# newton-physics/newton

Hardware: NVIDIA H100
Metric: env_steps_per_sec (higher is better)
Workload: dtype f32

## Files before the change

newton_b200/build.py:

```python

from __future__ import annotations

import os
import subprocess
import sys

HERE = os.path.dirname(os.path.abspath(__file__))
CSRC = os.path.join(HERE, "csrc")
LIB = os.path.join(HERE, "libnewton_b200.so")
LIB_FAST = os.path.join(HERE, "libnewton_b200_fast.so")
STRICT_FLAGS = ["-fmad=false", "-DNB2_STRICT_FP=1"]
SOURCES = ["nb2_api.cu", "nb2_collide.cu", "nb2_xpbd.cu", "nb2_featherstone.cu", "nb2_selection.cu", "nb2_peer.cu", "nb2_match.cu"]
NVCC_FLAGS = [
    "-gencode", "arch=compute_90a,code=sm_90a", "-lineinfo", "-O3", "-std=c++17", "--expt-relaxed-constexpr",
    "-Xcompiler", "-fPIC", "-Xcompiler", "-O2",
]


def _nvcc() -> str:
    for c in (os.environ.get("NVCC"), "/usr/local/cuda/bin/nvcc", "nvcc"):
        if c and (os.path.isabs(c) and os.path.exists(c) or not os.path.isabs(c)):
            return c
    return "nvcc"


def needs_build() -> bool:
    if not os.path.exists(LIB):
        return True
    t = os.path.getmtime(LIB)
    deps = [os.path.join(CSRC, f) for f in os.listdir(CSRC)] + [os.path.join(HERE, "..", "include", "newton_b200.h")]
    return any(os.path.getmtime(p) > t for p in deps)


def build(force: bool = False, verbose: bool = False) -> str:
    if not force and not needs_build() and os.path.exists(LIB_FAST):
        return LIB
    procs = []
    variants = ((LIB, ".o", STRICT_FLAGS), (LIB_FAST, ".fast.o", []))
    for _lib_path, suffix, extra in variants:
        flags = NVCC_FLAGS + extra
        if verbose:
            flags = flags + ["-Xptxas", "-v"]
        for src in SOURCES:
            obj = os.path.join(CSRC, src.replace(".cu", suffix))
            cmd = [_nvcc(), *flags, "-c", os.path.join(CSRC, src), "-o", obj]
            procs.append((src, subprocess.Popen(cmd, stdout=subprocess.PIPE, stderr=subprocess.STDOUT, text=True)))
    for src, p in procs:
        out, _ = p.communicate()
        if verbose or p.returncode != 0:
            sys.stderr.write(out)
        if p.returncode != 0:
            raise RuntimeError(f"nvcc failed on {src}")
    for lib_path, suffix, _extra in variants:
        objs = [os.path.join(CSRC, src.replace(".cu", suffix)) for src in SOURCES]
        subprocess.run([_nvcc(), "-shared", "-o", lib_path, *objs, "-lcudart"], check=True)
    return LIB


def build_variant(tag: str, defines: list[str], strict: bool = True, sources=None) -> str:
    lib_path = os.path.join(HERE, f"libnewton_b200_{tag}.so")
    flags = NVCC_FLAGS + (STRICT_FLAGS if strict else []) + list(defines)
    procs, objs = [], []
    for src in SOURCES:
        obj = os.path.join(CSRC, src.replace(".cu", f".{tag}.o"))
        objs.append(obj)
        procs.append((src, subprocess.Popen([_nvcc(), *flags, "-c", os.path.join(CSRC, src), "-o", obj], stdout=subprocess.PIPE,
                                            stderr=subprocess.STDOUT, text=True)))
    for src, p in procs:
        out, _ = p.communicate()
        if p.returncode != 0:
            sys.stderr.write(out)
            raise RuntimeError(f"nvcc failed on {src} ({tag})")
    subprocess.run([_nvcc(), "-shared", "-o", lib_path, *objs, "-lcudart"], check=True)
    return lib_path


if __name__ == "__main__":
    print(build(force=True, verbose="-v" in sys.argv))
```

newton_b200/csrc/nb2_api.cu:

```cuda
#include <algorithm>
#include <cstdlib>
#include <atomic>
#include <cstdio>
#include <cstring>
#include <mutex>

#include <cmath>

#include "nb2_internal.cuh"

namespace nb2 {

static thread_local std::string g_last_error;
static std::atomic<int64_t> g_launches{0};

void set_error(const std::string& msg) { g_last_error = msg; }
void count_launch(int n) { g_launches.fetch_add(n, std::memory_order_relaxed); }

template <typename T>
static nb2_status fetch(const T* dptr, size_t n, std::vector<T>& out) {
    out.resize(n);
    if (n == 0) return NB2_OK;
    if (!dptr) {
        set_error("nb2_model_create: required model array is NULL");
        return NB2_ERR_INVALID_ARGUMENT;
    }
    NB2_CUDA_CHECK(cudaMemcpy(out.data(), dptr, n * sizeof(T), cudaMemcpyDefault));
    return NB2_OK;
}

template <typename T>
static nb2_status upload(nb2_model* m, const std::vector<T>& v, const T** out) {
    void* p = nullptr;
    size_t bytes = std::max<size_t>(v.size(), 1) * sizeof(T);
    NB2_CUDA_CHECK(cudaMalloc(&p, bytes));
    m->allocations.push_back(p);
    if (!v.empty()) NB2_CUDA_CHECK(cudaMemcpy(p, v.data(), v.size() * sizeof(T), cudaMemcpyHostToDevice));
    *out = static_cast<const T*>(p);
    return NB2_OK;
}

static int pow2_at_least(int x) {
    int p = 1;
    while (p < x) p <<= 1;
    return p;
}

static nb2_status build_tables(nb2_model* m, const nb2_model_desc& d) {
    HostTables& h = m->host;
    const int W = d.world_count, B = d.body_count, J = d.joint_count, S = d.shape_count, P = d.shape_pair_count;
    if (W <= 0 || B < 0 || J < 0 || S < 0 || P < 0) {
        set_error("nb2_model_create: invalid counts");
        return NB2_ERR_INVALID_ARGUMENT;
    }
    std::vector<int> bws, jws, sws, shape_world, shape_type, shape_body, jparent, jchild, pairs, art_start, jart;
    nb2_status st;
    if ((st = fetch(d.body_world_start, size_t(W) + 2, bws))) return st;
    if ((st = fetch(d.joint_world_start, size_t(W) + 2, jws))) return st;
    if ((st = fetch(d.shape_world_start, size_t(W) + 2, sws))) return st;
    if ((st = fetch(d.shape_world, size_t(S), shape_world))) return st;
    if ((st = fetch(d.shape_type, size_t(S), shape_type))) return st;
    if ((st = fetch(d.shape_body, size_t(S), shape_body))) return st;
    if ((st = fetch(d.joint_parent, size_t(J), jparent))) return st;
    if ((st = fetch(d.joint_child, size_t(J), jchild))) return st;
    if ((st = fetch(d.shape_contact_pairs, size_t(P) * 2, pairs))) return st;
    if ((st = fetch(d.articulation_start, size_t(d.articulation_count) + 1, art_start))) return st;
    if ((st = fetch(d.joint_articulation, size_t(J), jart))) return st;
    std::vector<float> shape_scale;
    if ((st = fetch(d.shape_scale, size_t(S) * 3, shape_scale))) return st;

    const bool implicit_single = (W == 1) && (bws[0] == B) && (jws[0] == J) && (sws[0] == S);
    m->implicit_single = implicit_single;
    int E;
    h.global_shapes.clear();
    if (implicit_single) {
        E = 1;
        h.env_body_start = {0, B};
        h.env_joint_start = {0, J};
        h.env_shape_start = {0, S};
    } else {
        if (bws[0] != 0 || bws[W] != B || jws[0] != 0 || jws[W] != J) {
            set_error("bodies/joints in the global world (-1) of a multi-world model are not supported by the fused kernels");
            return NB2_ERR_UNSUPPORTED;
        }
        E = W;
        h.env_body_start.assign(bws.begin(), bws.begin() + W + 1);
        h.env_joint_start.assign(jws.begin(), jws.begin() + W + 1);
        h.env_shape_start.assign(sws.begin(), sws.begin() + W + 1);
        for (int s = 0; s < sws[0]; ++s) h.global_shapes.push_back(s);
        for (int s = sws[W]; s < S; ++s) h.global_shapes.push_back(s);
        for (int s : h.global_shapes)
            if (shape_body[s] != -1) {
                set_error("global (world -1) shapes must be static (body == -1)");
                return NB2_ERR_UNSUPPORTED;
            }
    }
    h.env_art_start.assign(size_t(E) + 1, 0);
    {
        int a = 0;
        for (int e = 0; e < E; ++e) {
            h.env_art_start[e] = a;
            while (a < d.articulation_count && art_start[a] < h.env_joint_start[e + 1]) ++a;
        }
        h.env_art_start[E] = d.articulation_count;
    }
    auto env_of_shape = [&](int s) -> int {
        if (implicit_single) return 0;
        return shape_world[s];
    };
    std::vector<int> hull_count;
    {
        bool any_mesh = false;
        for (int s = 0; s < S; ++s) any_mesh = any_mesh || shape_type[s] == 8;
        if (any_mesh) {
            if (!d.hull_points || !d.shape_hull_start || !d.shape_hull_count) {
                set_error("MESH shapes need model.hull_points / shape_hull_start / shape_hull_count (the mesh vertex pool)");
                return NB2_ERR_INVALID_ARGUMENT;
            }
            if ((st = fetch(d.shape_hull_count, size_t(S), hull_count))) return st;
        }
    }
    m->has_mesh_pairs = false;
    struct PairRec { int env; int64_t key; int sa, sb; int max_contacts; };
    std::vector<PairRec> recs;
    recs.reserve(P);
    for (int t = 0; t < P; ++t) {
        int s1 = pairs[2 * t], s2 = pairs[2 * t + 1];
        if (s1 < 0 || s2 < 0 || s1 >= S || s2 >= S || s1 == s2) continue;
        int w1 = env_of_shape(s1), w2 = env_of_shape(s2);
        int env = w1 >= 0 ? w1 : w2;
        if (w1 >= 0 && w2 >= 0 && w1 != w2) continue;
        if (env < 0) continue;
        int sa = s1, sb = s2, pair_max = 5;
        if (shape_type[sa] > shape_type[sb]) std::swap(sa, sb);
        {
            const int ta = shape_type[sa], tb = shape_type[sb];
            auto known = [](int t) { return t == 1 || (t >= 3 && t <= 10); };
            if (!known(ta) || !known(tb)) {
                set_error("shape pair (" + std::to_string(sa) + "," + std::to_string(sb) + "): geometry types " + std::to_string(ta) + "/" +
                          std::to_string(tb) + " are outside the supported set (plane, sphere, capsule, ellipsoid, cylinder, box, cone, "
                          "convex mesh)");
                return NB2_ERR_UNSUPPORTED;
            }
            if ((ta == 10 || tb == 10) &&
                (!d.hull_points || !d.shape_hull_start || !d.shape_hull_count || !d.shape_collision_aabb_lower || !d.shape_collision_aabb_upper)) {
                set_error("CONVEX_MESH shapes need model.hull_points / shape_hull_start / shape_hull_count / shape_collision_aabb_lower / _upper");
                return NB2_ERR_INVALID_ARGUMENT;
            }
            if (ta == 8 || tb == 8) {
                const bool infinite_plane_a = ta == 1 && shape_scale[3 * sa] == 0.0f && shape_scale[3 * sa + 1] == 0.0f;
                if (!(infinite_plane_a && tb == 8)) {
                    set_error("shape pair (" + std::to_string(sa) + "," + std::to_string(sb) + "): a MESH shape collides with infinite planes "
                              "only (one contact per vertex); mesh-mesh / mesh-convex / mesh-finite-plane need the reference's BVH / SDF "
                              "routes, which are out of scope - filter the pair or use a convex hull");
                    return NB2_ERR_UNSUPPORTED;
                }
                m->has_mesh_pairs = true;
                recs.push_back({env, ((int64_t(sb) & 0xFFFFF) << 43) | ((int64_t(sa) & 0xFFFFF) << 23), sb, sa, hull_count[sb]});
                continue;
            }
            {
                const bool early = ta >= 5 || tb == 9 || (ta == 4 && tb > 4);
                const bool barrel = tb == 6 && shape_scale[3 * sb + 2] != 0.0f;
                const bool analytic = !early && ((ta == 1 && (tb == 3 || tb == 4 || tb == 5 || (tb == 6 && !barrel) || tb == 7)) ||
                                                 (ta == 3 && (tb == 3 || tb == 4 || tb == 7 || (tb == 6 && !barrel))) || (ta == 4 && tb == 4));
                if (!analytic) m->has_convex_pairs = true;
                pair_max = analytic ? 4 : 5;
            }
        }
        int64_t key = ((int64_t(sa) & 0xFFFFF) << 43) | ((int64_t(sb) & 0xFFFFF) << 23);
        recs.push_back({env, key, sa, sb, pair_max});
    }
    std::stable_sort(recs.begin(), recs.end(), [](const PairRec& a, const PairRec& b) {
        return a.env != b.env ? a.env < b.env : a.key < b.key;
    });
    h.env_pair_start.assign(size_t(E) + 1, 0);
    h.env_slot_start.assign(size_t(E) + 1, 0);
    h.pairs.clear();
    h.pairs.reserve(recs.size());
    {
        size_t i = 0;
        for (int e = 0; e < E; ++e) {
            h.env_pair_start[e] = int(h.pairs.size());
            const int ss = h.env_shape_start[e], se = h.env_shape_start[e + 1];
            const int nloc = se - ss;
            auto slot_of = [&](int s) -> int {
                if (s >= ss && s < se) return s - ss;
                for (size_t g = 0; g < h.global_shapes.size(); ++g)
                    if (h.global_shapes[g] == s) return nloc + int(g);
                return -1;
            };
            int env_max = 0, env_slots = 0;
            for (; i < recs.size() && recs[i].env == e; ++i) {
                env_max += recs[i].max_contacts;
                m->max_env_contacts = std::max(m->max_env_contacts, env_max);
                int a = slot_of(recs[i].sa), b = slot_of(recs[i].sb);
                if (a < 0 || b < 0) {
                    set_error("contact pair references a shape outside its world");
                    return NB2_ERR_INVALID_ARGUMENT;
                }
                const bool mesh_pair = shape_type[recs[i].sa] == 8;
                h.pairs.push_back(make_int2(a, mesh_pair ? (b | NB2_PAIR_MESH_PLANE) : b));
                env_slots += mesh_pair ? recs[i].max_contacts : 5;
            }
            h.env_slot_start[e + 1] = h.env_slot_start[e] + env_slots;
        }
        h.env_pair_start[E] = int(h.pairs.size());
        h.explicit_env_slot_start = h.env_slot_start;
    }
    h.body_joint_start.assign(size_t(B) + 1, 0);
    for (int j = 0; j < J; ++j) {
        if (jparent[j] >= 0) h.body_joint_start[jparent[j] + 1]++;
        if (jchild[j] >= 0) h.body_joint_start[jchild[j] + 1]++;
    }
    for (int b = 0; b < B; ++b) h.body_joint_start[b + 1] += h.body_joint_start[b];
    h.body_joint_entry.assign(size_t(h.body_joint_start[B]), 0);
    {
        std::vector<int> fill(h.body_joint_start.begin(), h.body_joint_start.end() - 1);
        int e = 0;
        for (int j = 0; j < J; ++j) {
            while (e + 1 < E && j >= h.env_joint_start[e + 1]) ++e;
            int jl = j - h.env_joint_start[e];
            if (jparent[j] >= 0) h.body_joint_entry[fill[jparent[j]]++] = (jl << 1) | 0;
            if (jchild[j] >= 0) h.body_joint_entry[fill[jchild[j]]++] = (jl << 1) | 1;
            int bs = h.env_body_start[e], be = h.env_body_start[e + 1];
            if ((jparent[j] >= 0 && (jparent[j] < bs || jparent[j] >= be)) || jchild[j] < bs || jchild[j] >= be) {
                set_error("joint connects bodies of different worlds");
                return NB2_ERR_INVALID_ARGUMENT;
            }
        }
    }
    {
        std::vector<int> janc, jqd, bflags, jtype, jdim;
        if ((st = fetch(d.joint_ancestor, size_t(J), janc))) return st;
        if ((st = fetch(d.joint_type, size_t(J), jtype))) return st;
        if ((st = fetch(d.joint_dof_dim, size_t(J) * 2, jdim))) return st;
        if ((st = fetch(d.body_flags, size_t(B), bflags))) return st;
        for (int j = 0; j < J; ++j)
            if (jchild[j] != j) {
                h.featherstone_supported = false;
                h.featherstone_reason = "joint j must drive body j (the reference mass matrix assumes body index == joint index)";
            }
        if ((st = fetch(d.joint_qd_start, size_t(J) + 1, jqd))) return st;
        h.joint_depth.assign(size_t(J), 0);
        h.joint_anc_mask.assign(size_t(J), 0ull);
        h.art_H_start.assign(size_t(d.articulation_count) + 1, 0);
        h.env_H_start.assign(size_t(E) + 1, 0);
        int max_depth = 0;
        for (int a = 0; a < d.articulation_count; ++a) {
            const int j0 = art_start[a], j1 = art_start[a + 1];
            if (j1 - j0 > 64) {
                h.featherstone_supported = false;
                h.featherstone_reason = "articulations with more than 64 joints";
            }
            for (int j = j0; j < j1; ++j) {
                int anc = janc[j];
                if (anc >= j || (anc >= 0 && anc < j0)) {
                    h.featherstone_supported = false;
                    h.featherstone_reason = "joints must be stored parent-before-child inside their articulation";
                    h.fk_levels = false;
                    anc = -1;
                }
                h.joint_depth[j] = anc >= 0 ? h.joint_depth[anc] + 1 : 0;
                h.joint_anc_mask[j] = (anc >= 0 ? h.joint_anc_mask[anc] : 0ull) | (1ull << ((j - j0) & 63));
                max_depth = std::max(max_depth, h.joint_depth[j]);
                if (jart[j] != a) {
                    h.featherstone_supported = false;
                    h.featherstone_reason = "joints outside an articulation";
                }
            }
        }
        h.joint_desc_mask.assign(size_t(J), 0ull);
        h.dof_joint.assign(size_t(jqd[J]), 0);
        h.art_batch_count.assign(size_t(d.articulation_count), 0);
        h.art_hb_body_start.assign(size_t(d.articulation_count), 0);
        h.art_hb_row_start.assign(size_t(d.articulation_count), 0);
        h.hb_body_col.clear();
        h.hb_row_col.clear();
        for (int a = 0; a < d.articulation_count && h.featherstone_supported; ++a) {
            const int j0 = art_start[a], j1 = art_start[a + 1], anj = j1 - j0;
            const int ad0 = jqd[j0], n = jqd[j1] - ad0;
            h.max_art_dofs = std::max(h.max_art_dofs, n);
            if (n > 127) {
                h.featherstone_supported = false;
                h.featherstone_reason = "articulations with more than 127 dofs";
                break;
            }
            int maxdep = 0;
            for (int j = j0; j < j1; ++j) {
                maxdep = std::max(maxdep, h.joint_depth[j]);
                for (int k = jqd[j]; k < jqd[j + 1]; ++k) h.dof_joint[k] = (signed char)(j - j0);
                unsigned long long m = 0ull;
                for (int i = j0; i < j1; ++i) m |= ((h.joint_anc_mask[i] >> (j - j0)) & 1ull) << (i - j0);
                h.joint_desc_mask[j] = m;
            }
            auto anc_at = [&](int i, int dep) {
                int jb = -1;
                for (unsigned long long m = h.joint_anc_mask[j0 + i]; m; m &= m - 1ull) {
                    const int b = __builtin_ctzll(m);
                    if (h.joint_depth[j0 + b] == dep) jb = b;
                }
                return jb;
            };
            h.art_hb_body_start[a] = int(h.hb_body_col.size());
            h.art_hb_row_start[a] = int(h.hb_row_col.size());
            int batches = 0;
            for (int dep = 0; dep <= maxdep; ++dep)
                for (int kk = 0; kk < 6; ++kk) {
                    bool any = false;
                    for (int j = j0; j < j1 && !any; ++j) any = h.joint_depth[j] == dep && jqd[j + 1] - jqd[j] > kk;
                    if (!any) break;
                    for (int i = 0; i < anj; ++i) {
                        const int jb = h.joint_depth[j0 + i] >= dep ? anc_at(i, dep) : -1;
                        const bool on = jb >= 0 && jqd[j0 + jb + 1] - jqd[j0 + jb] > kk;
                        h.hb_body_col.push_back(on ? (signed char)(jqd[j0 + jb] - ad0 + kk) : (signed char)-1);
                    }
                    for (int ra = 0; ra < n; ++ra) {
                        const int ja = h.dof_joint[ad0 + ra];
                        const int jb = h.joint_depth[j0 + ja] >= dep ? anc_at(ja, dep) : -1;
                        int col = -1;
                        if (jb >= 0 && jqd[j0 + jb + 1] - jqd[j0 + jb] > kk) col = jqd[j0 + jb] - ad0 + kk;
                        if (col > ra) col = -1;
                        h.hb_row_col.push_back((signed char)col);
                    }
                    batches += 1;
                }
            h.art_batch_count[a] = batches;
        }
        {
            std::vector<char> driven(size_t(B), 0);
            for (int j = 0; j < J; ++j)
                if (jart[j] >= 0 && jchild[j] >= 0) {
                    if (driven[jchild[j]]) h.fk_levels = false;
                    driven[jchild[j]] = 1;
                }
        }
        int e = 0, max_env_H = 0, max_env_arts = 0;
        for (int ee = 0; ee < E; ++ee) {
            int acc = 0;
            for (int a = h.env_art_start[ee]; a < h.env_art_start[ee + 1]; ++a) {
                h.art_H_start[a] = acc;
                int nd = jqd[art_start[a + 1]] - jqd[art_start[a]];
                acc += nd * nd;
            }
            h.env_H_start[ee + 1] = h.env_H_start[ee] + acc;
            max_env_H = std::max(max_env_H, acc);
            max_env_arts = std::max(max_env_arts, h.env_art_start[ee + 1] - h.env_art_start[ee]);
        }
        (void)e;
        m->dev.max_depth = max_depth;
        m->dev.max_env_H = max_env_H;
        m->dev.max_env_arts = max_env_arts;
        int max_dofs = 0, max_coords = 0;
        std::vector<int> jq;
        if ((st = fetch(d.joint_q_start, size_t(J) + 1, jq))) return st;
        for (int ee = 0; ee < E; ++ee) {
            int ja = h.env_joint_start[ee], jb = h.env_joint_start[ee + 1];
            max_dofs = std::max(max_dofs, jqd[jb] - jqd[ja]);
            max_coords = std::max(max_coords, jq[jb] - jq[ja]);
        }
        m->dev.max_env_dofs = max_dofs;
        m->dev.max_env_coords = max_coords;
    }
    DevModel& dv = m->dev;
    dv.d = d;
    dv.env_count = E;
    dv.global_shape_count = int(h.global_shapes.size());
    dv.max_env_bodies = dv.max_env_joints = dv.max_env_slots_shapes = dv.max_env_pairs = dv.max_env_contact_slots = 0;
    for (int e = 0; e < E; ++e) {
        dv.max_env_bodies = std::max(dv.max_env_bodies, h.env_body_start[e + 1] - h.env_body_start[e]);
        dv.max_env_joints = std::max(dv.max_env_joints, h.env_joint_start[e + 1] - h.env_joint_start[e]);
        dv.max_env_slots_shapes =
            std::max(dv.max_env_slots_shapes, h.env_shape_start[e + 1] - h.env_shape_start[e] + dv.global_shape_count);
        dv.max_env_pairs = std::max(dv.max_env_pairs, h.env_pair_start[e + 1] - h.env_pair_start[e]);
        dv.max_env_contact_slots = std::max(dv.max_env_contact_slots, h.env_slot_start[e + 1] - h.env_slot_start[e]);
    }
    dv.slot_total = h.env_slot_start[E];
    dv.has_mesh_pairs = m->has_mesh_pairs ? 1 : 0;
    m->lanes_per_env =
        std::min(32, std::max(8, pow2_at_least(std::max({dv.max_env_bodies, dv.max_env_joints, std::min(dv.max_env_pairs, 32)}))));
    {
        int sms = 132;
        cudaDeviceGetAttribute(&sms, cudaDevAttrMultiProcessorCount, m->device);
        while (m->lanes_per_env < 32 && (long long)E * m->lanes_per_env / 32 < 4LL * sms) m->lanes_per_env *= 2;
    }
    if (const char* ov = std::getenv("NB2_LANES")) {
        const int v = std::atoi(ov);
        if (v == 8 || v == 16 || v == 32) m->lanes_per_env = v;
    }
    return NB2_OK;
}

static void free_allocations(nb2_model* m) {
    for (void* p : m->allocations) cudaFree(p);
    m->allocations.clear();
}

static nb2_status upload_tables(nb2_model* m) {
    HostTables& h = m->host;
    DevModel& dv = m->dev;
    nb2_status st;
    if ((st = upload(m, h.env_body_start, &dv.env_body_start))) return st;
    if ((st = upload(m, h.env_joint_start, &dv.env_joint_start))) return st;
    if ((st = upload(m, h.env_shape_start, &dv.env_shape_start))) return st;
    if ((st = upload(m, h.env_pair_start, &dv.env_pair_start))) return st;
    if ((st = upload(m, h.env_slot_start, &dv.env_slot_start))) return st;
    if ((st = upload(m, h.env_art_start, &dv.env_art_start))) return st;
    if ((st = upload(m, h.global_shapes, &dv.global_shapes))) return st;
    if ((st = upload(m, h.pairs, &dv.pairs))) return st;
    if ((st = upload(m, h.body_joint_start, &dv.body_joint_start))) return st;
    if ((st = upload(m, h.body_joint_entry, &dv.body_joint_entry))) return st;
    if ((st = upload(m, h.joint_depth, &dv.joint_depth))) return st;
    if ((st = upload(m, h.joint_anc_mask, &dv.joint_anc_mask))) return st;
    if ((st = upload(m, h.art_H_start, &dv.art_H_start))) return st;
    if ((st = upload(m, h.env_H_start, &dv.env_H_start))) return st;
    if ((st = upload(m, h.art_batch_count, &dv.art_batch_count))) return st;
    if ((st = upload(m, h.art_hb_body_start, &dv.art_hb_body_start))) return st;
    if ((st = upload(m, h.art_hb_row_start, &dv.art_hb_row_start))) return st;
    if ((st = upload(m, h.hb_body_col, &dv.hb_body_col))) return st;
    if ((st = upload(m, h.hb_row_col, &dv.hb_row_col))) return st;
    if ((st = upload(m, h.joint_desc_mask, &dv.joint_desc_mask))) return st;
    if ((st = upload(m, h.dof_joint, &dv.dof_joint))) return st;
    void* p = nullptr;
    {
        size_t nL = std::max<size_t>(size_t(h.env_H_start.back()), 1);
        NB2_CUDA_CHECK(cudaMalloc(&p, nL * sizeof(float)));
        NB2_CUDA_CHECK(cudaMemset(p, 0, nL * sizeof(float)));
        m->allocations.push_back(p);
        dv.fs_L = static_cast<float*>(p);
    }
    {
        size_t n = std::max<size_t>(size_t(dv.slot_total) * 6, 1) * sizeof(float);
        NB2_CUDA_CHECK(cudaMalloc(&p, n));
        NB2_CUDA_CHECK(cudaMemset(p, 0, n));
        m->allocations.push_back(p);
        dv.contact_impulse = static_cast<float*>(p);
        n = std::max<size_t>(size_t(dv.d.joint_count) * 6, 1) * sizeof(float);
        NB2_CUDA_CHECK(cudaMalloc(&p, n));
        NB2_CUDA_CHECK(cudaMemset(p, 0, n));
        m->allocations.push_back(p);
        dv.joint_impulse = static_cast<float*>(p);
    }
    size_t cb_bytes = std::max<size_t>(size_t(dv.slot_total) * CF_COUNT, 1) * sizeof(float);
    NB2_CUDA_CHECK(cudaMalloc(&p, cb_bytes));
    NB2_CUDA_CHECK(cudaMemset(p, 0, cb_bytes));
    m->allocations.push_back(p);
    dv.cb = static_cast<float*>(p);
    NB2_CUDA_CHECK(cudaMalloc(&p, (size_t(dv.env_count) + 1) * sizeof(int)));
    NB2_CUDA_CHECK(cudaMemset(p, 0, (size_t(dv.env_count) + 1) * sizeof(int)));
    m->allocations.push_back(p);
    dv.env_contact_count = static_cast<int*>(p);
    NB2_CUDA_CHECK(cudaMalloc(&p, (size_t(dv.env_count) + 1) * sizeof(int)));
    NB2_CUDA_CHECK(cudaMemset(p, 0, (size_t(dv.env_count) + 1) * sizeof(int)));
    m->allocations.push_back(p);
    dv.env_contact_offset = static_cast<int*>(p);
    NB2_CUDA_CHECK(cudaMalloc(&p, 4 * sizeof(int)));
    const int sync_init[4] = {0, 0, 1, 0};
    NB2_CUDA_CHECK(cudaMemcpy(p, sync_init, sizeof(sync_init), cudaMemcpyHostToDevice));
    m->allocations.push_back(p);
    dv.collide_sync = static_cast<int*>(p);
    NB2_CUDA_CHECK(cudaMalloc(&p, std::max<size_t>(size_t(dv.env_count), 1) * sizeof(unsigned long long)));
    NB2_CUDA_CHECK(cudaMemset(p, 0, std::max<size_t>(size_t(dv.env_count), 1) * sizeof(unsigned long long)));
    m->allocations.push_back(p);
    dv.collide_tile_status = static_cast<unsigned long long*>(p);
    return NB2_OK;
}


static void release(nb2_model* m, const void* p) {
    if (!p) return;
    for (size_t i = 0; i < m->allocations.size(); ++i)
        if (m->allocations[i] == p) {
            cudaFree(m->allocations[i]);
            m->allocations.erase(m->allocations.begin() + i);
            return;
        }
}

static nb2_status allocate_contact_blocks(nb2_model* m) {
    DevModel& dv = m->dev;
    HostTables& h = m->host;
    const int E = dv.env_count;
    release(m, dv.env_slot_start);
    release(m, dv.cb);
    release(m, dv.contact_impulse);
    dv.max_env_contact_slots = 0;
    for (int e = 0; e < E; ++e) dv.max_env_contact_slots = std::max(dv.max_env_contact_slots, h.env_slot_start[e + 1] - h.env_slot_start[e]);
    dv.slot_total = h.env_slot_start[E];
    nb2_status st;
    if ((st = upload(m, h.env_slot_start, &dv.env_slot_start))) return st;
    void* p = nullptr;
    size_t n = std::max<size_t>(size_t(dv.slot_total) * 6, 1) * sizeof(float);
    NB2_CUDA_CHECK(cudaMalloc(&p, n));
    NB2_CUDA_CHECK(cudaMemset(p, 0, n));
    m->allocations.push_back(p);
    dv.contact_impulse = static_cast<float*>(p);
    n = std::max<size_t>(size_t(dv.slot_total) * CF_COUNT, 1) * sizeof(float);
    NB2_CUDA_CHECK(cudaMalloc(&p, n));
    NB2_CUDA_CHECK(cudaMemset(p, 0, n));
    m->allocations.push_back(p);
    dv.cb = static_cast<float*>(p);
    NB2_CUDA_CHECK(cudaMemset(dv.env_contact_count, 0, (size_t(E) + 1) * sizeof(int)));
    return NB2_OK;
}

static nb2_status configure_broad_phase(nb2_model* m, int mode, int max_pairs, bool include_static_kinematic) {
    DevModel& dv = m->dev;
    HostTables& h = m->host;
    const int E = dv.env_count;
    dv.include_static_kinematic_pairs = include_static_kinematic ? 1 : 0;
    if (mode == dv.broad_phase && (mode == NB2_BROAD_PHASE_EXPLICIT || max_pairs == m->dyn_pairs_requested)) return NB2_OK;
    release(m, dv.dyn_pairs);
    release(m, dv.env_dyn_count);
    dv.dyn_pairs = nullptr;
    dv.env_dyn_count = nullptr;
    dv.dyn_pair_cap = 0;
    if (mode != NB2_BROAD_PHASE_EXPLICIT && m->has_mesh_pairs) {
        set_error("nb2_collide_configure: MESH shapes are supported with the explicit broad phase only");
        return NB2_ERR_UNSUPPORTED;
    }
    if (mode == NB2_BROAD_PHASE_EXPLICIT) {
        h.env_slot_start = h.explicit_env_slot_start;
        m->max_env_contacts = m->explicit_max_env_contacts;
        m->has_convex_pairs = m->explicit_has_convex_pairs;
    } else {
        if (dv.max_env_slots_shapes > 65535) {
            set_error("nb2_collide_configure: more than 65535 shapes in one world");
            return NB2_ERR_CAPACITY;
        }
        if (!dv.d.shape_collision_group) {
            set_error("nb2_collide_configure: broad_phase nxn / sap needs model.shape_collision_group");
            return NB2_ERR_INVALID_ARGUMENT;
        }
        int cap = 0;
        std::vector<int> caps(size_t(E), 0);
        for (int e = 0; e < E; ++e) {
            const long long ns = h.env_shape_start[e + 1] - h.env_shape_start[e] + dv.global_shape_count;
            long long c = ns * (ns - 1) / 2;
            if (max_pairs > 0) c = std::min<long long>(c, max_pairs);
            caps[e] = int(std::min<long long>(c, 1 << 20));
            cap = std::max(cap, caps[e]);
        }
        for (int e = 0; e < E; ++e) h.env_slot_start[e + 1] = h.env_slot_start[e] + 5 * caps[e];
        if (h.env_slot_start[E] < 0 || (long long)E * cap > (1ll << 30)) {
            set_error("nb2_collide_configure: candidate capacity too large; pass max_pairs_per_world (CollisionPipeline(shape_pairs_max=...))");
            return NB2_ERR_CAPACITY;
        }
        dv.dyn_pair_cap = cap;
        void* p = nullptr;
        NB2_CUDA_CHECK(cudaMalloc(&p, std::max<size_t>(size_t(E) * cap, 1) * sizeof(int2)));
        m->allocations.push_back(p);
        dv.dyn_pairs = static_cast<int2*>(p);
        NB2_CUDA_CHECK(cudaMalloc(&p, (size_t(E) + 1) * sizeof(int)));
        NB2_CUDA_CHECK(cudaMemset(p, 0, (size_t(E) + 1) * sizeof(int)));
        m->allocations.push_back(p);
        dv.env_dyn_count = static_cast<int*>(p);
        m->max_env_contacts = 5 * cap;
        m->has_convex_pairs = true;
        release(m, dv.filter_keys);
        dv.filter_keys = nullptr;
        dv.filter_count = 0;
        if (dv.d.shape_collision_filter_pair_count > 0 && dv.d.shape_collision_filter_pairs) {
            std::vector<int> fp;
            nb2_status st = fetch(dv.d.shape_collision_filter_pairs, size_t(dv.d.shape_collision_filter_pair_count) * 2, fp);
            if (st != NB2_OK) return st;
            std::vector<long long> keys;
            keys.reserve(fp.size() / 2);
            for (size_t i = 0; i + 1 < fp.size(); i += 2) {
                const long long a = std::min(fp[i], fp[i + 1]), b = std::max(fp[i], fp[i + 1]);
                keys.push_back((a << 32) | b);
            }
            std::sort(keys.begin(), keys.end());
            keys.erase(std::unique(keys.begin(), keys.end()), keys.end());
            const long long* dk = nullptr;
            if ((st = upload(m, keys, &dk))) return st;
            dv.filter_keys = dk;
            dv.filter_count = int(keys.size());
        }
    }
    dv.broad_phase = mode;
    m->dyn_pairs_requested = max_pairs;
    return allocate_contact_blocks(m);
}

struct DeviceGuard {
    int prev = -1, dev = -1;
    explicit DeviceGuard(int device) : dev(device) {
        if (cudaGetDevice(&prev) != cudaSuccess) prev = -1;
        if (prev != dev) cudaSetDevice(dev);
    }
    ~DeviceGuard() {
        if (prev >= 0 && prev != dev) cudaSetDevice(prev);
    }
};

}

using namespace nb2;

extern "C" {

nb2_status nb2_model_create(const nb2_model_desc* desc, int32_t device, nb2_model** out) {
    if (!desc || !out) {
        set_error("nb2_model_create: NULL argument");
        return NB2_ERR_INVALID_ARGUMENT;
    }
    *out = nullptr;
    DeviceGuard guard(device);
    nb2_model* m = new nb2_model();
    m->device = device;
    nb2_status st = build_tables(m, *desc);
    if (st == NB2_OK) st = upload_tables(m);
    if (st != NB2_OK) {
        free_allocations(m);
        delete m;
        return st;
    }
    m->explicit_max_env_contacts = m->max_env_contacts;
    m->explicit_has_convex_pairs = m->has_convex_pairs;
    m->dev.include_static_kinematic_pairs = 1;
    *out = m;
    return NB2_OK;
}

void nb2_model_destroy(nb2_model* model) {
    if (!model) return;
    DeviceGuard guard(model->device);
    for (void* p : {(void*)model->match_new_keys, (void*)model->match_prev_keys, (void*)model->match_prev_claim, (void*)model->match_prev_pos,
                    (void*)model->match_prev_normal, (void*)model->match_prev_count, (void*)model->match_prev_record,
                    (void*)model->match_prev_was_matched})
        if (p) cudaFree(p);
    free_allocations(model);
    delete model;
}

nb2_status nb2_model_notify_changed(nb2_model* model, const nb2_model_desc* desc, int32_t flags) {
    (void)flags;
    if (!model || !desc) {
        set_error("nb2_model_notify_changed: NULL argument");
        return NB2_ERR_INVALID_ARGUMENT;
    }
    const nb2_model_desc& o = model->dev.d;
    if (desc->body_count != o.body_count || desc->joint_count != o.joint_count || desc->shape_count != o.shape_count ||
        desc->shape_pair_count != o.shape_pair_count || desc->world_count != o.world_count ||
        desc->articulation_count != o.articulation_count || desc->joint_dof_count != o.joint_dof_count ||
        desc->joint_coord_count != o.joint_coord_count || desc->gravity_count != o.gravity_count) {
        set_error("nb2_model_notify_changed: topology changed; create a new nb2_model");
        return NB2_ERR_UNSUPPORTED;
    }
    model->dev.d = *desc;
    return NB2_OK;
}

int32_t nb2_model_rigid_contact_max(const nb2_model* model) { return model ? model->dev.slot_total : 0; }

nb2_status nb2_collide_configure(nb2_model* model, int32_t broad_phase, int32_t max_pairs_per_world, int32_t include_static_kinematic_pairs) {
    if (!model || broad_phase < NB2_BROAD_PHASE_EXPLICIT || broad_phase > NB2_BROAD_PHASE_SAP || max_pairs_per_world < 0) {
        set_error("nb2_collide_configure: invalid argument");
        return NB2_ERR_INVALID_ARGUMENT;
    }
    DeviceGuard guard(model->device);
    return configure_broad_phase(model, broad_phase, max_pairs_per_world, include_static_kinematic_pairs != 0);
}

nb2_status nb2_collide(nb2_model* model, const float* body_q, const nb2_contacts_view* contacts, void* cuda_stream) {
    if (!model || (!body_q && model->dev.d.body_count > 0)) {
        set_error("nb2_collide: NULL argument");
        return NB2_ERR_INVALID_ARGUMENT;
    }
    model->dev.export_rank = nullptr;
    model->contacts_imported = false;
    model->dev.spec_mode = 0;
    model->dev.spec_body_qd = nullptr;
    model->dev.spec_dt = model->dev.spec_max_ext = 0.0f;
    DeviceGuard guard(model->device);
    return launch_collide(model, body_q, contacts, static_cast<cudaStream_t>(cuda_stream));
}

nb2_status nb2_collide_speculative(nb2_model* model, const float* body_q, const float* body_qd, float dt, float max_speculative_extension,
                                   const nb2_contacts_view* contacts, void* cuda_stream) {
    if (!model || ((!body_q || !body_qd) && model->dev.d.body_count > 0)) {
        set_error("nb2_collide_speculative: NULL argument");
        return NB2_ERR_INVALID_ARGUMENT;
    }
    if (!(dt >= 0.0f) || !(max_speculative_extension >= 0.0f) || std::isinf(dt) || std::isinf(max_speculative_extension)) {
        set_error("nb2_collide_speculative: dt and max_speculative_extension must be non-negative finite numbers");
        return NB2_ERR_INVALID_ARGUMENT;
    }
    if (!model->dev.d.shape_collision_aabb_lower || !model->dev.d.shape_collision_aabb_upper || !model->dev.d.body_com) {
        set_error("nb2_collide_speculative: model.shape_collision_aabb_lower / _upper / body_com are required");
        return NB2_ERR_INVALID_ARGUMENT;
    }
    model->dev.export_rank = nullptr;
    model->contacts_imported = false;
    model->dev.spec_mode = (dt > 0.0f && max_speculative_extension > 0.0f) ? 2 : 1;
    model->dev.spec_body_qd = body_qd;
    model->dev.spec_dt = dt;
    model->dev.spec_max_ext = max_speculative_extension;
    DeviceGuard guard(model->device);
    const nb2_status st = launch_collide(model, body_q, contacts, static_cast<cudaStream_t>(cuda_stream));
    model->dev.spec_mode = 0;
    model->dev.spec_body_qd = nullptr;
    return st;
}

nb2_status nb2_contacts_sort(nb2_model* model, const nb2_contacts_view* c, void* cuda_stream) {
    if (!model || !c || !c->rigid_contact_count || !c->shape0 || !c->shape1 || !c->point0 || !c->point1 || !c->offset0 || !c->offset1 ||
        !c->normal || !c->margin0 || !c->margin1 || c->rigid_contact_max < 0) {
        set_error("nb2_contacts_sort: NULL argument / contacts view has NULL arrays");
        return NB2_ERR_INVALID_ARGUMENT;
    }
    DeviceGuard guard(model->device);
    return launch_contacts_sort(model, *c, static_cast<cudaStream_t>(cuda_stream));
}

nb2_status nb2_contacts_import(nb2_model* model, const nb2_contacts_view* c, void* cuda_stream) {
    if (!model || !c || !c->rigid_contact_count || !c->shape0 || !c->shape1 || !c->point0 || !c->point1 || !c->offset0 || !c->offset1 ||
        !c->normal || !c->margin0 || !c->margin1 || c->rigid_contact_max < 0) {
        set_error("nb2_contacts_import: NULL argument / contacts view has NULL arrays");
        return NB2_ERR_INVALID_ARGUMENT;
    }
    DeviceGuard guard(model->device);
    model->contacts_imported = true;
    return launch_contacts_import(model, *c, static_cast<cudaStream_t>(cuda_stream));
}

nb2_status nb2_xpbd_step(nb2_model* model, const nb2_xpbd_params* params, const nb2_state_view* state_in,
                         const nb2_state_view* state_out, const nb2_control_view* control, int32_t use_contacts, float dt,
                         void* cuda_stream) {
    if (!model || !params || !state_in || !state_out || !control) {
        set_error("nb2_xpbd_step: NULL argument");
        return NB2_ERR_INVALID_ARGUMENT;
    }
    if (params->iterations < 0 || !(dt > 0.0f)) {
        set_error("nb2_xpbd_step: iterations must be >= 0 and dt > 0");
        return NB2_ERR_INVALID_ARGUMENT;
    }
    if ((use_contacts & NB2_XPBD_CONTACT_IMPULSE) && (use_contacts & NB2_XPBD_USE_CONTACTS)) model->xpbd_impulse_dt = dt;
    DeviceGuard guard(model->device);
    return launch_xpbd_step(model, *params, *state_in, *state_out, *control, use_contacts, dt,
                            static_cast<cudaStream_t>(cuda_stream));
}

nb2_status nb2_xpbd_update_contacts(nb2_model* model, const nb2_contacts_view* contacts, void* cuda_stream) {
    if (!model || !contacts || !contacts->force || !contacts->rigid_contact_count) {
        set_error("nb2_xpbd_update_contacts: NULL argument (contacts.force must be allocated)");
        return NB2_ERR_INVALID_ARGUMENT;
    }
    if (!(model->xpbd_impulse_dt > 0.0f)) {
        set_error("nb2_xpbd_update_contacts: no contact impulse data available, run nb2_xpbd_step with NB2_XPBD_CONTACT_IMPULSE first");
        return NB2_ERR_INVALID_ARGUMENT;
    }
    DeviceGuard guard(model->device);
    return launch_xpbd_update_contacts(model, *contacts, static_cast<cudaStream_t>(cuda_stream));
}

nb2_status nb2_integrate_bodies(nb2_model* model, const nb2_state_view* state_in, const nb2_state_view* state_out,
                                float angular_damping, float dt, void* cuda_stream) {
    if (!model || !state_in || !state_out) {
        set_error("nb2_integrate_bodies: NULL argument");
        return NB2_ERR_INVALID_ARGUMENT;
    }
    DeviceGuard guard(model->device);
    return launch_integrate_bodies(model, *state_in, *state_out, angular_damping, dt, static_cast<cudaStream_t>(cuda_stream));
}

nb2_status nb2_featherstone_step(nb2_model* model, const nb2_featherstone_params* params, const nb2_state_view* state_in,
                                 const nb2_state_view* state_out, const nb2_control_view* control, int32_t use_contacts,
                                 float dt, void* cuda_stream) {
    if (!model || !params || !state_in || !state_out || !control) {
        set_error("nb2_featherstone_step: NULL argument");
        return NB2_ERR_INVALID_ARGUMENT;
    }
    DeviceGuard guard(model->device);
    return launch_featherstone_step(model, *params, *state_in, *state_out, *control, use_contacts, dt,
                                    static_cast<cudaStream_t>(cuda_stream));
}

nb2_status nb2_eval_fk(nb2_model* model, const float* joint_q, const float* joint_qd, float* body_q, float* body_qd,
                       void* cuda_stream) {
    if (!model || !joint_q || !joint_qd || !body_q || !body_qd) {
        set_error("nb2_eval_fk: NULL argument");
        return NB2_ERR_INVALID_ARGUMENT;
    }
    DeviceGuard guard(model->device);
    return launch_eval_fk(model, joint_q, joint_qd, body_q, body_qd, static_cast<cudaStream_t>(cuda_stream));
}

nb2_status nb2_eval_fk_masked(nb2_model* model, const float* joint_q, const float* joint_qd, float* body_q, float* body_qd,
                              const uint8_t* articulation_mask, const int32_t* articulation_indices, int32_t index_count,
                              int32_t body_flag_filter, void* cuda_stream) {
    if (!model || !joint_q || !joint_qd || !body_q || !body_qd) {
        set_error("nb2_eval_fk_masked: NULL argument");
        return NB2_ERR_INVALID_ARGUMENT;
    }
    if (articulation_mask && articulation_indices) {
        set_error("nb2_eval_fk_masked: cannot specify both mask and indices");
        return NB2_ERR_INVALID_ARGUMENT;
    }
    if (articulation_indices && index_count < 0) {
        set_error("nb2_eval_fk_masked: negative index_count");
        return NB2_ERR_INVALID_ARGUMENT;
    }
    DeviceGuard guard(model->device);
    return launch_eval_fk(model, joint_q, joint_qd, body_q, body_qd, static_cast<cudaStream_t>(cuda_stream), articulation_mask,
                          articulation_indices, index_count, body_flag_filter);
}

nb2_status nb2_eval_ik(nb2_model* model, const float* body_q, const float* body_qd, float* joint_q, float* joint_qd,
                       void* cuda_stream) {
    if (!model || !body_q || !body_qd || !joint_q || !joint_qd) {
        set_error("nb2_eval_ik: NULL argument");
        return NB2_ERR_INVALID_ARGUMENT;
    }
    DeviceGuard guard(model->device);
    return launch_eval_ik(model, body_q, body_qd, joint_q, joint_qd, static_cast<cudaStream_t>(cuda_stream));
}

const char* nb2_last_error(void) { return g_last_error.c_str(); }
int64_t nb2_kernel_launch_count(void) { return g_launches.load(std::memory_order_relaxed); }
const char* nb2_version(void) { return "newton_b200 0.1 (sm_90a)"; }

}
```

newton_b200/csrc/nb2_internal.cuh:

```cuda
#pragma once
#include <cuda_runtime.h>
#include <stdint.h>

#include <string>
#include <vector>

#include "../../include/newton_b200.h"

namespace nb2 {

enum ContactField {
    CF_BODY_A = 0,
    CF_BODY_B,
    CF_SHAPE0,
    CF_SHAPE1,
    CF_P0X, CF_P0Y, CF_P0Z,
    CF_P1X, CF_P1Y, CF_P1Z,
    CF_O0X, CF_O0Y, CF_O0Z,
    CF_O1X, CF_O1Y, CF_O1Z,
    CF_NX, CF_NY, CF_NZ,
    CF_MARGIN0, CF_MARGIN1,
    CF_MU, CF_MU_TORSIONAL, CF_MU_ROLLING,
    CF_KE, CF_KD, CF_KF, CF_KA,
    CF_COUNT
};

struct DevModel {
    nb2_model_desc d;
    int env_count;
    const int* env_body_start;
    const int* env_joint_start;
    const int* env_shape_start;
    const int* env_pair_start;
    const int* env_slot_start;
    const int* env_art_start;
    const int* global_shapes;
    int global_shape_count;
    const int2* pairs;
    const int* body_joint_start;
    const int* body_joint_entry;
    float* cb;
    int slot_total;
    int* env_contact_count;
    int* env_contact_offset;
    int* collide_sync;
    unsigned long long* collide_tile_status;
    int max_env_bodies, max_env_joints, max_env_slots_shapes, max_env_pairs, max_env_contact_slots;
    const int* joint_depth;
    const unsigned long long* joint_anc_mask;
    const int* art_H_start;
    const int* env_H_start;
    float* fs_L;
    int max_depth, max_env_dofs, max_env_coords, max_env_H, max_env_arts;
    const int* art_batch_count;
    const int* art_hb_body_start;
    const int* art_hb_row_start;
    const signed char* hb_body_col;
    const signed char* hb_row_col;
    const unsigned long long* joint_desc_mask;
    const signed char* dof_joint;
    float* contact_impulse;
    float* joint_impulse;
    const int* export_rank;
    int broad_phase;
    int include_static_kinematic_pairs;
    int dyn_pair_cap;
    int2* dyn_pairs;
    int* env_dyn_count;
    const long long* filter_keys;
    int filter_count;
    int lane_per_contact;
    int spec_mode;
    int has_mesh_pairs;
    const float* spec_body_qd;
    float spec_dt, spec_max_ext;
};

enum : int { NB2_PAIR_MESH_PLANE = 0x40000000 };

struct HostTables {
    std::vector<int> env_body_start, env_joint_start, env_shape_start, env_pair_start, env_slot_start, env_art_start;
    std::vector<int> explicit_env_slot_start;
    std::vector<int> global_shapes;
    std::vector<int2> pairs;
    std::vector<int> body_joint_start, body_joint_entry;
    std::vector<int> joint_depth, art_H_start, env_H_start;
    std::vector<unsigned long long> joint_anc_mask, joint_desc_mask;
    std::vector<int> art_batch_count, art_hb_body_start, art_hb_row_start;
    std::vector<signed char> hb_body_col, hb_row_col, dof_joint;
    int max_art_dofs = 0;
    bool featherstone_supported = true;
    bool fk_levels = true;
    std::string featherstone_reason;
};

}

struct nb2_model {
    int device = 0;
    nb2::DevModel dev{};
    nb2::HostTables host;
    std::vector<void*> allocations;
    int lanes_per_env = 32;
    int featherstone_step_count = 0;
    int import_capacity = 0;
    int *import_keys = nullptr, *import_keys_sorted = nullptr, *import_idx = nullptr, *import_idx_sorted = nullptr;
    void* import_temp = nullptr;
    size_t import_temp_bytes = 0;
    int sort_capacity = 0;
    unsigned long long *sort_keys = nullptr, *sort_keys_sorted = nullptr;
    int *sort_idx = nullptr, *sort_idx_sorted = nullptr;
    float* sort_stage = nullptr;
    int* sort_rank = nullptr;
    void* sort_temp = nullptr;
    size_t sort_temp_bytes = 0;
    int match_capacity = 0;
    long long *match_new_keys = nullptr, *match_prev_keys = nullptr, *match_prev_claim = nullptr;
    float *match_prev_pos = nullptr, *match_prev_normal = nullptr;
    int* match_prev_count = nullptr;
    float* match_prev_record = nullptr;
    int* match_prev_was_matched = nullptr;
    bool match_prev_has_record = false;
    bool implicit_single = false;
    bool has_convex_pairs = false;
    bool has_mesh_pairs = false;
    int explicit_max_env_contacts = 0, dyn_pairs_requested = 0;
    bool explicit_has_convex_pairs = false;
    int max_env_contacts = 0;
    bool contacts_imported = false;
    float xpbd_impulse_dt = 0.0f;
};

namespace nb2 {
void set_error(const std::string& msg);
void count_launch(int n = 1);
nb2_status launch_collide(nb2_model* m, const float* body_q, const nb2_contacts_view* contacts, cudaStream_t s);
nb2_status launch_broadphase(nb2_model* m, const float* body_q, cudaStream_t s);
nb2_status launch_xpbd_step(nb2_model* m, const nb2_xpbd_params& p, const nb2_state_view& in, const nb2_state_view& out,
                            const nb2_control_view& ctl, int use_contacts, float dt, cudaStream_t s);
nb2_status launch_contacts_sort(nb2_model* m, const nb2_contacts_view& contacts, cudaStream_t s);
nb2_status launch_contacts_import(nb2_model* m, const nb2_contacts_view& contacts, cudaStream_t s);
nb2_status launch_xpbd_update_contacts(nb2_model* m, const nb2_contacts_view& contacts, cudaStream_t s);
nb2_status launch_integrate_bodies(nb2_model* m, const nb2_state_view& in, const nb2_state_view& out, float angular_damping,
                                   float dt, cudaStream_t s);
nb2_status launch_featherstone_step(nb2_model* m, const nb2_featherstone_params& p, const nb2_state_view& in,
                                    const nb2_state_view& out, const nb2_control_view& ctl, int use_contacts, float dt,
                                    cudaStream_t s);
nb2_status launch_eval_fk(nb2_model* m, const float* joint_q, const float* joint_qd, float* body_q, float* body_qd,
                          cudaStream_t s, const uint8_t* mask = nullptr, const int* indices = nullptr, int index_count = 0,
                          int body_flag_filter = 3);
nb2_status launch_eval_ik(nb2_model* m, const float* body_q, const float* body_qd, float* joint_q, float* joint_qd, cudaStream_t s);
}

#define NB2_CUDA_CHECK(expr)                                                                          \
    do {                                                                                              \
        cudaError_t _e = (expr);                                                                      \
        if (_e != cudaSuccess) {                                                                      \
            nb2::set_error(std::string(#expr) + ": " + cudaGetErrorString(_e));                       \
            return NB2_ERR_CUDA;                                                                      \
        }                                                                                             \
    } while (0)
```

newton_b200/csrc/nb2_xpbd.cu:

```cuda
#include <cstdlib>

#include "nb2_internal.cuh"
#include "nb2_math.cuh"

#define NB2_GPU __device__ __forceinline__

namespace nb2 {

enum { JT_PRISMATIC = 0, JT_REVOLUTE = 1, JT_BALL = 2, JT_FIXED = 3, JT_FREE = 4, JT_DISTANCE = 5, JT_D6 = 6, JT_ROD = 7 };
enum { BODY_KINEMATIC = 2 };

enum { BR_Q = 0, BR_QD = 7, BR_COM = 13, BR_INVM = 16, BR_INVI = 17, BR_I = 26, BR_SIZE = 35 };
enum { DR_SIZE = 13 };
enum { XF_JOINT_CACHE = 1, XF_TMA = 2, XF_PHASE_SYNC = 4, XF_PHASE_SYNC_FINE = 8 };
enum { CC_P0 = 0, CC_P1 = 3, CC_N = 6, CC_MSUM = 9, CC_MU = 10, CC_MUT = 11, CC_MUR = 12, CC_Q0 = 13, CC_Q1 = 16, CC_SIZE = 19 };

#ifdef NB2_XPBD_NOINLINE
#define NB2_HELPER __host__ __device__ __noinline__
#else
#define NB2_HELPER NB2_DEV
#endif
#ifndef NB2_XPBD_ROLLED
#define NB2_ROW_UNROLL _Pragma("unroll")
#else
#define NB2_ROW_UNROLL _Pragma("unroll 1")
#endif

struct BodyView {
    Xf X;
    V3 com;
    float inv_m;
    const float* rec;
    V3 v, w;
};

NB2_DEV BodyView load_body(const float* rec) {
    BodyView b;
    b.X = ldx(rec + BR_Q);
    b.v = ld3(rec + BR_QD);
    b.w = ld3(rec + BR_QD + 3);
    b.com = ld3(rec + BR_COM);
    b.inv_m = rec[BR_INVM];
    b.rec = rec;
    return b;
}
NB2_DEV BodyView static_body() {
    BodyView b;
    b.inv_m = 0.f;
    b.rec = nullptr;
    return b;
}

NB2_HELPER float ang_inv_mass(const float* rec, V3 ang) {
    if (rec == nullptr) return 0.0f;
    const Q4 q(rec[BR_Q + 3], rec[BR_Q + 4], rec[BR_Q + 5], rec[BR_Q + 6]);
    const V3 r = qrot_inv(q, ang);
    return dot(r, mv(ldm(rec + BR_INVI), r));
}

NB2_DEV float generalized_inv_mass(const BodyView& a, const BodyView& b, V3 lin_a, V3 lin_b, V3 ang_a, V3 ang_b) {
    float denom = 0.0f;
    denom += len2(lin_a) * a.inv_m;
    denom += len2(lin_b) * b.inv_m;
    denom += ang_inv_mass(a.rec, ang_a);
    denom += ang_inv_mass(b.rec, ang_b);
    return denom;
}
NB2_DEV float contact_delta(float err, const BodyView& a, const BodyView& b, V3 lin_a, V3 lin_b, V3 ang_a, V3 ang_b, float relaxation,
                            float dt) {
    float denom = generalized_inv_mass(a, b, lin_a, lin_b, ang_a, ang_b);
    float dl = -err;
    if (denom > 0.0f) dl /= dt * denom;
    return dl * relaxation;
}
NB2_DEV float positional_correction(float err, float derr, const BodyView& a, const BodyView& b, V3 lin_a, V3 lin_b, V3 ang_a, V3 ang_b,
                                    float compliance, float damping, float dt) {
    float denom = generalized_inv_mass(a, b, lin_a, lin_b, ang_a, ang_b);
    float alpha = compliance, gamma = compliance * damping;
    float dl = -(err + alpha * 0.0f + gamma * derr);
    if (denom + alpha > 0.0f) dl /= (dt + gamma) * denom + alpha / dt;
    return dl;
}
NB2_DEV float angular_correction(float err, float derr, const BodyView& a, const BodyView& b, V3 ang_a, V3 ang_b, float compliance,
                                 float damping, float dt) {
    float denom = 0.0f;
    denom += ang_inv_mass(a.rec, ang_a);
    denom += ang_inv_mass(b.rec, ang_b);
    float alpha = compliance, gamma = compliance * damping;
    float dl = -(err + alpha * 0.0f + gamma * derr);
    if (denom + alpha > 0.0f) dl /= (dt + gamma) * denom + alpha / dt;
    return dl;
}

struct AxisSetup {
    V3 lim_lo, lim_up, target_pos, stiffness, target_vel, damping;
};
NB2_DEV AxisSetup gather_axes(const nb2_model_desc& d, const nb2_control_view& ctl, int axis_start, int target_start, int offset,
                              int count) {
    AxisSetup s;
    V3 pos_t, pos_w, vel_t, vel_w;
#pragma unroll
    for (int k = 0; k < 3; ++k) {
        if (count > k) {
            int ai = axis_start + offset + k, ti = target_start + offset + k;
            V3 axis = ld3(d.joint_axis + 3 * ai);
            V3 lo_t = axis * d.joint_limit_lower[ai], up_t = axis * d.joint_limit_upper[ai];
            V3 lo = vmin(lo_t, up_t), up = vmax(lo_t, up_t);
            if (k == 0) {
                s.lim_lo = lo;
                s.lim_up = up;
            } else {
                s.lim_lo = vmin(s.lim_lo, lo);
                s.lim_up = vmax(s.lim_up, up);
            }
            float ke = d.joint_target_ke[ai], kd = d.joint_target_kd[ai];
            if (ke > 0.0f) {
                V3 wa = axis * ke;
                pos_t += wa * ctl.joint_target_q[ti];
                pos_w += vabs(wa);
            }
            if (kd > 0.0f) {
                V3 wa = axis * kd;
                vel_t += wa * ctl.joint_target_qd[ai];
                vel_w += vabs(wa);
            }
        }
    }
    s.target_pos = pos_t;
    s.stiffness = pos_w;
    s.target_vel = vel_t;
    s.damping = vel_w;
    if (s.stiffness.x > 0.0f) s.target_pos.x /= s.stiffness.x;
    if (s.stiffness.y > 0.0f) s.target_pos.y /= s.stiffness.y;
    if (s.stiffness.z > 0.0f) s.target_pos.z /= s.stiffness.z;
    if (s.damping.x > 0.0f) s.target_vel.x /= s.damping.x;
    if (s.damping.y > 0.0f) s.target_vel.y /= s.damping.y;
    if (s.damping.z > 0.0f) s.target_vel.z /= s.damping.z;
    return s;
}

struct Deltas {
    V3 lin_p, ang_p, lin_c, ang_c;
};

enum { JC_XP = 0, JC_XC = 7, JC_ANG = 14, JC_HDR = 32, JC_CHILD = 33, JC_PARENT = 34, JC_AXIS = 35, JC_TARGET = 36,
       JC_SIZE = 37 };
NB2_DEV int jc_int(const float* jc, int k) { return reinterpret_cast<const int*>(jc)[k]; }
NB2_DEV void store_axis_setup(float* p, const AxisSetup& s) {
    st3(p, s.lim_lo); st3(p + 3, s.lim_up); st3(p + 6, s.target_pos); st3(p + 9, s.stiffness); st3(p + 12, s.target_vel); st3(p + 15, s.damping);
}
NB2_DEV AxisSetup load_axis_setup(const float* p) {
    AxisSetup s;
    s.lim_lo = ld3(p); s.lim_up = ld3(p + 3); s.target_pos = ld3(p + 6); s.stiffness = ld3(p + 9); s.target_vel = ld3(p + 12); s.damping = ld3(p + 15);
    return s;
}

NB2_DEV bool solve_joint(const nb2_model_desc& d, const nb2_control_view& ctl, const nb2_xpbd_params& P, int j, int body0,
                         const float* bodies, const float* jc, float dt, Deltas& out) {
    const int hdr = jc ? jc_int(jc, JC_HDR)
                       : (d.joint_type[j] | (d.joint_enabled[j] ? 16 : 0) | (d.joint_dof_dim[2 * j] << 8) | (d.joint_dof_dim[2 * j + 1] << 12));
    const int type = hdr & 15;
    if (!(hdr & 16) || type == JT_FREE) return false;
    const int id_c = (jc ? jc_int(jc, JC_CHILD) : d.joint_child[j]) - body0;
    const int id_p_raw = jc ? jc_int(jc, JC_PARENT) : d.joint_parent[j];
    const int id_p = id_p_raw >= 0 ? id_p_raw - body0 : -1;
    const Xf X_pj = jc ? ldx(jc + JC_XP) : ldx(d.joint_X_p + 7 * j), X_cj = jc ? ldx(jc + JC_XC) : ldx(d.joint_X_c + 7 * j);
    BodyView bp = static_body();
    Xf X_wp = X_pj;
    Xf pose_p = X_pj;
    if (id_p >= 0) {
        bp = load_body(bodies + id_p * BR_SIZE);
        pose_p = bp.X;
        X_wp = xmul(pose_p, X_wp);
    } else {
        bp.X = pose_p;
    }
    BodyView bc = load_body(bodies + id_c * BR_SIZE);
    const Xf pose_c = bc.X;
    const Xf X_wc = xmul(pose_c, X_cj);
    if (bp.inv_m == 0.0f && bc.inv_m == 0.0f) return false;
    V3 lin_dp, ang_dp, lin_dc, ang_dc;
    const Xf rel_pose = xmul(xinv(X_wp), X_wc);
    const V3 rel_p = rel_pose.p;
    const V3 x_p = X_wp.p, x_c = X_wc.p;
    const int axis_start = jc ? jc_int(jc, JC_AXIS) : d.joint_qd_start[j];
    const int target_start = jc ? jc_int(jc, JC_TARGET) : d.joint_target_q_start[j];
    const int lin_count = (hdr >> 8) & 15, ang_count = (hdr >> 12) & 15;
    const V3 wcom_p = xpoint(pose_p, bp.com);
    const V3 wcom_c = xpoint(pose_c, bc.com);
    const V3 vel_p = bp.v, omega_p = bp.w, vel_c = bc.v, omega_c = bc.w;

    if (type == JT_DISTANCE) {
        V3 r_p = x_p - wcom_p, r_c = x_c - wcom_c;
        float lower = d.joint_limit_lower[axis_start], upper = d.joint_limit_upper[axis_start];
        if (lower < 0.0f && upper < 0.0f) return false;
        V3 ad = x_c - x_p;
        float dist = len(ad);
        float err = 0.0f;
        if (lower >= 0.0f && dist < lower) err = dist - lower;
        else if (upper >= 0.0f && dist > upper) err = dist - upper;
        if (fabsf(err) > 1e-9f) {
            V3 lc;
            if (dist > 1e-9f) lc = ad / dist;
            else {
                V3 cd = wcom_c - wcom_p;
                lc = len2(cd) > 1e-18f ? unit(cd) : xvec(X_wp, V3(1.f, 0.f, 0.f));
            }
            V3 lp = -lc, ap = -cross(r_p, lc), ac = cross(r_c, lc);
            float derr = dot(lp, vel_p) + dot(lc, vel_c) + dot(ap, omega_p) + dot(ac, omega_c);
            float compliance = P.joint_linear_compliance;
            float ke = d.joint_target_ke[axis_start];
            if (ke > 0.0f) compliance = 1.0f / ke;
            float damping = d.joint_target_kd[axis_start];
            float dl = positional_correction(err, derr, bp, bc, lp, lc, ap, ac, compliance, damping, dt);
            lin_dp += lp * (dl * P.joint_linear_relaxation);
            ang_dp += ap * (dl * P.joint_angular_relaxation);
            lin_dc += lc * (dl * P.joint_linear_relaxation);
            ang_dc += ac * (dl * P.joint_angular_relaxation);
        }
    } else {
        const AxisSetup s = gather_axes(d, ctl, axis_start, target_start, 0, lin_count);
        V3 proj = rel_p;
#pragma unroll
        for (int dim = 0; dim < 3; ++dim) {
            float lo = s.lim_lo.get(dim), up = s.lim_up.get(dim), e = rel_p.get(dim);
            if (e < lo) proj.set(dim, lo);
            else if (e > up) proj.set(dim, up);
            else if (s.stiffness.get(dim) > 0.0f) proj.set(dim, clamp_w(s.target_pos.get(dim), lo, up));
        }
        const V3 r_p = xpoint(X_wp, proj) - wcom_p;
        const V3 r_c = x_c - wcom_c;
        NB2_ROW_UNROLL
        for (int dim = 0; dim < 3; ++dim) {
            float e = rel_p.get(dim);
            V3 lc = qrot(X_wp.q, V3(dim == 0 ? 1.f : 0.f, dim == 1 ? 1.f : 0.f, dim == 2 ? 1.f : 0.f));
            V3 lp = -lc, ap = -cross(r_p, lc), ac = cross(r_c, lc);
            float derr = dot(lp, vel_p) + dot(lc, vel_c) + dot(ap, omega_p) + dot(ac, omega_c);
            float err = 0.0f, compliance = P.joint_linear_compliance, damping = 0.0f;
            float derr_rel = derr - s.target_vel.get(dim);
            float lo = s.lim_lo.get(dim), up = s.lim_up.get(dim);
            if (e < lo) err = e - lo;
            else if (e > up) err = e - up;
            else {
                float tp = clamp_w(s.target_pos.get(dim), lo, up);
                float ks = s.stiffness.get(dim), kdm = s.damping.get(dim);
                if (ks > 0.0f) {
                    err = e - tp;
                    compliance = 1.0f / ks;
                    damping = kdm;
                } else if (kdm > 0.0f) {
                    compliance = 1.0f / kdm;
                    damping = kdm;
                }
            }
            if (fabsf(err) > 1e-9f || fabsf(derr_rel) > 1e-9f) {
                float dl = positional_correction(err, derr_rel, bp, bc, lp, lc, ap, ac, compliance, damping, dt);
                lin_dp += lp * (dl * P.joint_linear_relaxation);
                ang_dp += ap * (dl * P.joint_angular_relaxation);
                lin_dc += lc * (dl * P.joint_linear_relaxation);
                ang_dc += ac * (dl * P.joint_angular_relaxation);
            }
        }
    }

    if (type == JT_FIXED || type == JT_PRISMATIC || type == JT_REVOLUTE || type == JT_D6) {
        const Q4 q_p = X_wp.q;
        Q4 q_c = X_wc.q;
        if (qdot(q_p, q_c) < 0.0f) q_c = qscale(q_c, -1.0f);
        const Q4 rq = qmul(qconj(q_p), q_c);
        const Q4 qtwist = qunit(Q4(rq.x, 0.0f, 0.0f, rq.w));
        const Q4 qswing = qmul(rq, qconj(qtwist));
        const float sn = sqrtf(rq.x * rq.x + rq.w * rq.w);
        const float invs = 1.0f / sn;
        const float invscube = invs * invs * invs;
        float err_0 = 2.0f * asin_w(clamp_w(qtwist.x, -1.0f, 1.0f));
        float err_1 = qswing.y, err_2 = qswing.z;
        Q4 g0(invs - rq.x * rq.x * invscube, 0.0f, 0.0f, -(rq.w * rq.x) * invscube);
        Q4 g1(-rq.w * (rq.w * rq.z + rq.x * rq.y) * invscube, rq.w * invs, -rq.x * invs, rq.x * (rq.w * rq.z + rq.x * rq.y) * invscube);
        Q4 g2(rq.w * (rq.w * rq.y - rq.x * rq.z) * invscube, rq.x * invs, rq.w * invs, rq.x * (rq.z * rq.x - rq.w * rq.y) * invscube);
        g0 = qscale(g0, 2.0f / fabsf(qtwist.w));
        const float swing_sq = qswing.w * qswing.w;
        if (swing_sq + 1.0e-4f < 1.0f) {
            float dd = sqrtf(1.0f - qswing.w * qswing.w);
            float theta = 2.0f * acos_w(clamp_w(qswing.w, -1.0f, 1.0f));
            float scale = theta / dd;
            err_1 *= scale;
            err_2 *= scale;
            g1 = qscale(g1, scale);
            g2 = qscale(g2, scale);
        }
        const AxisSetup s = jc ? load_axis_setup(jc + JC_ANG) : gather_axes(d, ctl, axis_start, target_start, lin_count, ang_count);
        const Q4 qc_inv = qconj(q_c);
        NB2_ROW_UNROLL
        for (int dim = 0; dim < 3; ++dim) {
            float e = dim == 0 ? err_0 : (dim == 1 ? err_1 : err_2);
            Q4 grad = dim == 0 ? g0 : (dim == 1 ? g1 : g2);
            Q4 quat_c = qmul(qmul(qscale(q_p, 0.5f), grad), qc_inv);
            V3 ac(quat_c.x, quat_c.y, quat_c.z);
            V3 ap = -ac;
            float derr = dot(ap, omega_p) + dot(ac, omega_c);
            float err = 0.0f, compliance = P.joint_angular_compliance, damping = 0.0f;
            float derr_rel = derr - s.target_vel.get(dim) * len(ac);
            float lo = s.lim_lo.get(dim), up = s.lim_up.get(dim);
            if (e < lo) err = e - lo;
            else if (e > up) err = e - up;
            else {
                float tp = clamp_w(s.target_pos.get(dim), lo, up);
                float ks = s.stiffness.get(dim), kdm = s.damping.get(dim);
                if (ks > 0.0f) {
                    err = e - tp;
                    compliance = 1.0f / ks;
                    damping = kdm;
                } else if (kdm > 0.0f) {
                    damping = kdm;
                    compliance = 1.0f / kdm;
                }
            }
            float dl = angular_correction(err, derr_rel, bp, bc, ap, ac, compliance, damping, dt) * P.joint_angular_relaxation;
            ang_dp += ap * dl;
            ang_dc += ac * dl;
        }
    }
    out.lin_p = lin_dp;
    out.ang_p = ang_dp;
    out.lin_c = lin_dc;
    out.ang_c = ang_dc;
    return true;
}

NB2_DEV bool joint_force_wrench(const nb2_model_desc& d, const float* joint_f, int j, int body0, const float* bodies, Deltas& out) {
    const int type = d.joint_type[j];
    if (!d.joint_enabled[j] || type == JT_FIXED || type == JT_ROD) return false;
    const int qd_start = d.joint_qd_start[j];
    const int lin_count = d.joint_dof_dim[2 * j], ang_count = d.joint_dof_dim[2 * j + 1];
    const int ndof = (type == JT_FREE || type == JT_DISTANCE) ? 6 : (type == JT_BALL ? 3 : lin_count + ang_count);
    bool any = false;
    for (int k = 0; k < ndof; ++k) any |= joint_f[qd_start + k] != 0.0f;
    if (!any) return false;
    const int id_c = d.joint_child[j] - body0;
    const int id_p_raw = d.joint_parent[j];
    const int id_p = id_p_raw >= 0 ? id_p_raw - body0 : -1;
    V3 f_total, t_total;
    if (type == JT_FREE || type == JT_DISTANCE) {
        f_total = V3(joint_f[qd_start], joint_f[qd_start + 1], joint_f[qd_start + 2]);
        t_total = V3(joint_f[qd_start + 3], joint_f[qd_start + 4], joint_f[qd_start + 5]);
        out.lin_p = f_total;
        out.ang_p = t_total;
        out.lin_c = f_total;
        out.ang_c = t_total;
        return true;
    }
    const Xf X_pj = ldx(d.joint_X_p + 7 * j), X_cj = ldx(d.joint_X_c + 7 * j);
    Xf X_wp = X_pj, pose_p = X_pj;
    V3 com_p;
    if (id_p >= 0) {
        pose_p = ldx(bodies + id_p * BR_SIZE + BR_Q);
        X_wp = xmul(pose_p, X_wp);
        com_p = ld3(bodies + id_p * BR_SIZE + BR_COM);
    }
    V3 r_p = X_wp.p - xpoint(pose_p, com_p);
    Xf pose_c = ldx(bodies + id_c * BR_SIZE + BR_Q);
    Xf X_wc = xmul(pose_c, X_cj);
    V3 r_c = X_wc.p - xpoint(pose_c, ld3(bodies + id_c * BR_SIZE + BR_COM));
    if (type == JT_BALL) {
        t_total = V3(joint_f[qd_start], joint_f[qd_start + 1], joint_f[qd_start + 2]);
    } else {
        for (int k = 0; k < 3; ++k)
            if (lin_count > k) f_total += joint_f[qd_start + k] * xvec(X_wp, ld3(d.joint_axis + 3 * (qd_start + k)));
        for (int k = 0; k < 3; ++k)
            if (ang_count > k)
                t_total += joint_f[qd_start + lin_count + k] * xvec(X_wp, ld3(d.joint_axis + 3 * (qd_start + lin_count + k)));
    }
    out.lin_p = f_total;
    out.ang_p = t_total + cross(r_p, f_total);
    out.lin_c = f_total;
    out.ang_c = t_total + cross(r_c, f_total);
    return true;
}

NB2_DEV void store_deltas(float* rec, const Deltas& dl, float active) {
    st3(rec + 0, dl.lin_p);
    st3(rec + 3, dl.ang_p);
    st3(rec + 6, dl.lin_c);
    st3(rec + 9, dl.ang_c);
    rec[12] = active;
}

NB2_HELPER void apply_delta(float* rec, V3 dlin, V3 dang, float inv_weight, bool weighted, float dt) {
    const float inv_m = rec[BR_INVM];
    if (inv_m == 0.0f) return;
    const M33 inv_I = ldm(rec + BR_INVI), I = ldm(rec + BR_I);
    const V3 p0 = ld3(rec + BR_Q);
    const Q4 q0(rec[BR_Q + 3], rec[BR_Q + 4], rec[BR_Q + 5], rec[BR_Q + 6]);
    const V3 v0 = ld3(rec + BR_QD), w0 = ld3(rec + BR_QD + 3);
    float weight = 1.0f;
    if (weighted && inv_weight > 0.0f) weight = 1.0f / inv_weight;
    const V3 dp = dlin * (inv_m * weight);
    const V3 dq = dang * weight;
    const V3 wb = qrot_inv(q0, w0);
    const V3 dwb = mv(inv_I, qrot_inv(q0, dq));
    const V3 tb = cross(dwb, mv(I, wb + dwb)) + cross(wb, mv(I, dwb));
    const V3 dw1 = qrot(q0, dwb - mv(mscale(dt, inv_I), tb));
    const V3 h = dw1 * dt;
    Q4 q1 = qadd(q0, qmul(qscale(Q4(h.x, h.y, h.z, 0.0f), 0.5f), q0));
    q1 = qunit(q1);
    const V3 com = ld3(rec + BR_COM);
    const V3 x_com = p0 + qrot(q0, com);
    V3 p1 = x_com + dp * dt;
    p1 -= qrot(q1, com);
    V3 v1 = v0 + dp, w1 = w0 + dw1;
    if (len(v1) < 1e-4f) v1 = V3();
    if (len(w1) < 1e-4f) w1 = V3();
    st3(rec + BR_Q, p1);
    rec[BR_Q + 3] = q1.x; rec[BR_Q + 4] = q1.y; rec[BR_Q + 5] = q1.z; rec[BR_Q + 6] = q1.w;
    st3(rec + BR_QD, v1);
    st3(rec + BR_QD + 3, w1);
}

NB2_GPU unsigned smem_u32(const void* p) { return static_cast<unsigned>(__cvta_generic_to_shared(p)); }
NB2_GPU void mbar_init(unsigned long long* bar, int count) {
    asm volatile("mbarrier.init.shared::cta.b64 [%0], %1;" ::"r"(smem_u32(bar)), "r"(count) : "memory");
    asm volatile("fence.mbarrier_init.release.cluster;" ::: "memory");
}
NB2_GPU void mbar_expect_tx(unsigned long long* bar, unsigned bytes) {
    asm volatile("mbarrier.arrive.expect_tx.shared::cta.b64 _, [%0], %1;" ::"r"(smem_u32(bar)), "r"(bytes) : "memory");
}
NB2_GPU void mbar_wait(unsigned long long* bar, unsigned parity) {
    unsigned done = 0;
    while (!done)
        asm volatile("{ .reg .pred p; mbarrier.try_wait.parity.shared::cta.b64 p, [%1], %2; selp.u32 %0, 1, 0, p; }"
                     : "=r"(done) : "r"(smem_u32(bar)), "r"(parity) : "memory");
}
NB2_GPU void bulk_g2s(void* dst_smem, const void* src_gmem, unsigned bytes, unsigned long long* bar) {
    asm volatile("cp.async.bulk.shared::cluster.global.mbarrier::complete_tx::bytes [%0], [%1], %2, [%3];"
                 ::"r"(smem_u32(dst_smem)), "l"(src_gmem), "r"(bytes), "r"(smem_u32(bar)) : "memory");
}
NB2_GPU void bulk_s2g(void* dst_gmem, const void* src_smem, unsigned bytes) {
    asm volatile("cp.async.bulk.global.shared::cta.bulk_group [%0], [%1], %2;" ::"l"(dst_gmem), "r"(smem_u32(src_smem)), "r"(bytes) : "memory");
}
NB2_GPU void bulk_commit_and_drain() {
    asm volatile("cp.async.bulk.commit_group;" ::: "memory");
    asm volatile("cp.async.bulk.wait_group.read 0;" ::: "memory");
}
NB2_GPU void fence_async_smem() { asm volatile("fence.proxy.async.shared::cta;" ::: "memory"); }

struct XpbdPlan {
    int bodies, jcache, cpair, ccache, extra, drec, mbar, total;
    int rec_cap;
};
__host__ __device__ inline XpbdPlan xpbd_plan(int NE, int MB, int MJ, int CC, bool ex, bool joint_cache, int contact_cache = 0) {
    XpbdPlan o;
    auto up4 = [](int x) { return (x + 3) & ~3; };
    o.rec_cap = MB > MJ ? (MB > CC ? MB : CC) : (MJ > CC ? MJ : CC);
    o.bodies = 0;
    o.jcache = up4(o.bodies + NE * MB * BR_SIZE);
    o.cpair = up4(o.jcache + (joint_cache ? NE * MJ * JC_SIZE : 0));
    o.ccache = up4(o.cpair + NE * CC);
    o.extra = up4(o.ccache + NE * contact_cache * CC_SIZE);
    o.drec = up4(o.extra + (ex ? NE * MB * 14 : 0));
    o.mbar = up4(o.drec + NE * o.rec_cap * DR_SIZE);
    o.total = o.mbar + 4;
    return o;
}
enum { ST_Q = 0, ST_QD = 7, ST_COM = 13, ST_INVM = 16, ST_I = 17, ST_INVI = 26, ST_PER_BODY = 35 };

#ifndef NB2_XPBD_MIN_WARPS
#define NB2_XPBD_MIN_WARPS 16
#endif
template <int L, bool EX, int WARPS>
__global__ void __launch_bounds__(32 * WARPS, (WARPS >= NB2_XPBD_MIN_WARPS ? 1 : NB2_XPBD_MIN_WARPS / WARPS))
xpbd_step_kernel(DevModel M, nb2_xpbd_params P, nb2_state_view sin, nb2_state_view sout, nb2_control_view ctl, int use_contacts_flags,
                 float dt, int flags, int contact_cap, int contact_cache) {
    const int use_contacts = use_contacts_flags & NB2_XPBD_USE_CONTACTS;
    const bool want_cimp = EX && use_contacts && (use_contacts_flags & NB2_XPBD_CONTACT_IMPULSE);
    const bool want_jimp = EX && sout.body_parent_f != nullptr;
    const bool want_init = EX && (P.enable_restitution || P.compute_body_velocity_from_position_delta);
    const bool joint_cache = (flags & XF_JOINT_CACHE) != 0;
    constexpr int G = 32 / L;
    constexpr int NE = G * WARPS;
    extern __shared__ __align__(16) float smem[];
    const int lane = threadIdx.x & 31, warp = threadIdx.x >> 5;
    const int grp = lane / L, l = lane % L;
    const int slot = warp * G + grp;
    const int env0 = blockIdx.x * NE;
    if (env0 >= M.env_count) return;
    const int env = env0 + slot;
    const bool live = env < M.env_count;
    const nb2_model_desc& d = M.d;
    const XpbdPlan plan = xpbd_plan(NE, M.max_env_bodies, M.max_env_joints, contact_cap, EX, joint_cache, contact_cache);
    float* ccache = smem + plan.ccache + slot * contact_cache * CC_SIZE;
    float* bodies = smem + plan.bodies + slot * M.max_env_bodies * BR_SIZE;
    float* drec = smem + plan.drec + slot * plan.rec_cap * DR_SIZE;
    int* cpair = reinterpret_cast<int*>(smem + plan.cpair) + slot * contact_cap;
    float* init_qd = smem + plan.extra + slot * M.max_env_bodies * 14;
    float* bcnt = init_qd + M.max_env_bodies * 13;
    float* jcache = joint_cache ? smem + plan.jcache + slot * M.max_env_joints * JC_SIZE : nullptr;
    float* stage = smem + plan.drec;
    unsigned long long* mbar = reinterpret_cast<unsigned long long*>(smem + plan.mbar);

    int b0 = 0, nb = 0, j0 = 0, nj = 0, slot0 = 0, nc = 0;
    if (live) {
        b0 = M.env_body_start[env];
        nb = M.env_body_start[env + 1] - b0;
        j0 = M.env_joint_start[env];
        nj = M.env_joint_start[env + 1] - j0;
        slot0 = M.env_slot_start[env];
        nc = use_contacts ? min(M.env_contact_count[env], contact_cap) : 0;
    }
    const int env_last = min(env0 + NE, M.env_count);
    const int cb0 = M.env_body_start[env0], cnb = M.env_body_start[env_last] - cb0;
    bool tma = (flags & XF_TMA) != 0 && cnb > 0 && (cb0 & 3) == 0 && (cnb & 3) == 0 && cnb * ST_PER_BODY <= NE * plan.rec_cap * DR_SIZE;
    if (tma) {
        const uintptr_t a = reinterpret_cast<uintptr_t>(sin.body_q) | reinterpret_cast<uintptr_t>(sin.body_qd) |
                            reinterpret_cast<uintptr_t>(sout.body_q) | reinterpret_cast<uintptr_t>(sout.body_qd) |
                            reinterpret_cast<uintptr_t>(d.body_com) | reinterpret_cast<uintptr_t>(d.body_inv_mass) |
                            reinterpret_cast<uintptr_t>(d.body_inertia) | reinterpret_cast<uintptr_t>(d.body_inv_inertia);
        tma = (a & 15) == 0;
    }
    if (tma) {
        if (threadIdx.x == 0) mbar_init(mbar, 1);
        __syncthreads();
        if (threadIdx.x == 0) {
            mbar_expect_tx(mbar, unsigned(cnb) * ST_PER_BODY * 4u);
            bulk_g2s(stage + ST_Q * cnb, sin.body_q + 7 * size_t(cb0), unsigned(cnb) * 28u, mbar);
            bulk_g2s(stage + ST_QD * cnb, sin.body_qd + 6 * size_t(cb0), unsigned(cnb) * 24u, mbar);
            bulk_g2s(stage + ST_COM * cnb, d.body_com + 3 * size_t(cb0), unsigned(cnb) * 12u, mbar);
            bulk_g2s(stage + ST_INVM * cnb, d.body_inv_mass + size_t(cb0), unsigned(cnb) * 4u, mbar);
            bulk_g2s(stage + ST_I * cnb, d.body_inertia + 9 * size_t(cb0), unsigned(cnb) * 36u, mbar);
            bulk_g2s(stage + ST_INVI * cnb, d.body_inv_inertia + 9 * size_t(cb0), unsigned(cnb) * 36u, mbar);
        }
    }
    for (int c = l; c < nc; c += L) {
        const size_t T = size_t(M.slot_total);
        int ba = __float_as_int(M.cb[CF_BODY_A * T + slot0 + c]), bb = __float_as_int(M.cb[CF_BODY_B * T + slot0 + c]);
        const unsigned ka = ba >= 0 && (d.body_flags[b0 + ba] & BODY_KINEMATIC) != 0, kb = bb >= 0 && (d.body_flags[b0 + bb] & BODY_KINEMATIC) != 0;
        cpair[c] = int(unsigned(ba + 1) | (ka << 15) | (unsigned(bb + 1) << 16) | (kb << 31));
        if (c < contact_cache) {
            const int s = slot0 + c;
            float* cc = ccache + c * CC_SIZE;
            const V3 p0(M.cb[CF_P0X * T + s], M.cb[CF_P0Y * T + s], M.cb[CF_P0Z * T + s]);
            const V3 p1(M.cb[CF_P1X * T + s], M.cb[CF_P1Y * T + s], M.cb[CF_P1Z * T + s]);
            const V3 o0(M.cb[CF_O0X * T + s], M.cb[CF_O0Y * T + s], M.cb[CF_O0Z * T + s]);
            const V3 o1(M.cb[CF_O1X * T + s], M.cb[CF_O1Y * T + s], M.cb[CF_O1Z * T + s]);
            st3(cc + CC_P0, p0);
            st3(cc + CC_P1, p1);
            st3(cc + CC_N, V3(M.cb[CF_NX * T + s], M.cb[CF_NY * T + s], M.cb[CF_NZ * T + s]));
            cc[CC_MSUM] = M.cb[CF_MARGIN0 * T + s] + M.cb[CF_MARGIN1 * T + s];
            cc[CC_MU] = M.cb[CF_MU * T + s];
            cc[CC_MUT] = M.cb[CF_MU_TORSIONAL * T + s];
            cc[CC_MUR] = M.cb[CF_MU_ROLLING * T + s];
            st3(cc + CC_Q0, p0 + o0);
            st3(cc + CC_Q1, p1 + o1);
        }
        if (want_cimp)
#pragma unroll
            for (int k = 0; k < 6; ++k) M.contact_impulse[k * T + slot0 + c] = 0.0f;
    }
    if (jcache)
        for (int j = l; j < nj; j += L) {
            const int gj = j0 + j;
            float* jc = jcache + j * JC_SIZE;
            const int lin_count = d.joint_dof_dim[2 * gj], ang_count = d.joint_dof_dim[2 * gj + 1];
            const int axis_start = d.joint_qd_start[gj], target_start = d.joint_target_q_start[gj];
            stx(jc + JC_XP, ldx(d.joint_X_p + 7 * gj));
            stx(jc + JC_XC, ldx(d.joint_X_c + 7 * gj));
            store_axis_setup(jc + JC_ANG, gather_axes(d, ctl, axis_start, target_start, lin_count, ang_count));
            jc[JC_HDR] = __int_as_float(d.joint_type[gj] | (d.joint_enabled[gj] ? 16 : 0) | (lin_count << 8) | (ang_count << 12));
            jc[JC_CHILD] = __int_as_float(d.joint_child[gj]);
            jc[JC_PARENT] = __int_as_float(d.joint_parent[gj]);
            jc[JC_AXIS] = __int_as_float(axis_start);
            jc[JC_TARGET] = __int_as_float(target_start);
        }
    if (tma) mbar_wait(mbar, 0);
    for (int b = l; b < nb; b += L) {
        const int gb = b0 + b;
        float* rec = bodies + b * BR_SIZE;
        const bool kin = (d.body_flags[gb] & BODY_KINEMATIC) != 0;
        if (tma) {
            const int sb = gb - cb0;
#pragma unroll
            for (int k = 0; k < 7; ++k) rec[BR_Q + k] = stage[ST_Q * cnb + 7 * sb + k];
#pragma unroll
            for (int k = 0; k < 6; ++k) rec[BR_QD + k] = stage[ST_QD * cnb + 6 * sb + k];
#pragma unroll
            for (int k = 0; k < 3; ++k) rec[BR_COM + k] = stage[ST_COM * cnb + 3 * sb + k];
            rec[BR_INVM] = kin ? 0.0f : stage[ST_INVM * cnb + sb];
#pragma unroll
            for (int k = 0; k < 9; ++k) {
                rec[BR_INVI + k] = kin ? 0.0f : stage[ST_INVI * cnb + 9 * sb + k];
                rec[BR_I + k] = stage[ST_I * cnb + 9 * sb + k];
            }
        } else {
#pragma unroll
            for (int k = 0; k < 7; ++k) rec[BR_Q + k] = sin.body_q[7 * gb + k];
#pragma unroll
            for (int k = 0; k < 6; ++k) rec[BR_QD + k] = sin.body_qd[6 * gb + k];
#pragma unroll
            for (int k = 0; k < 3; ++k) rec[BR_COM + k] = d.body_com[3 * gb + k];
            rec[BR_INVM] = kin ? 0.0f : d.body_inv_mass[gb];
#pragma unroll
            for (int k = 0; k < 9; ++k) {
                rec[BR_INVI + k] = kin ? 0.0f : d.body_inv_inertia[9 * gb + k];
                rec[BR_I + k] = d.body_inertia[9 * gb + k];
            }
        }
    }
    if (want_init)
        for (int b = l; b < nb; b += L)
#pragma unroll
            for (int k = 0; k < 13; ++k) init_qd[b * 13 + k] = bodies[b * BR_SIZE + BR_Q + k];
    if (tma) __syncthreads();
    else __syncwarp();
    const bool use_masks = nb <= L && nc <= 64;
    unsigned long long mask_a = 0ull, mask_b = 0ull;
    if (use_masks && l < nb)
        for (int c = 0; c < nc; ++c) {
            const int pr = cpair[c];
            const int ba = int(unsigned(pr) & 0x7fffu) - 1, bb = int((unsigned(pr) >> 16) & 0x7fffu) - 1;
            if (ba == bb) continue;
            if (ba == l) mask_a |= 1ull << c;
            if (bb == l) mask_b |= 1ull << c;
        }
    for (int j = l; j < nj; j += L) {
        Deltas w;
        bool act = joint_force_wrench(d, ctl.joint_f, j0 + j, b0, bodies, w);
        if (!act) w = Deltas();
        store_deltas(drec + j * DR_SIZE, w, act ? 1.0f : 0.0f);
        if (want_jimp) {
            float* ji = M.joint_impulse + 6 * size_t(j0 + j);
            const V3 a = V3() + w.lin_c * dt, t = V3() + w.ang_c * dt;
            st3(ji, a);
            st3(ji + 3, t);
        }
    }
    __syncwarp();
    for (int b = l; b < nb; b += L) {
        const int gb = b0 + b;
        float* rec = bodies + b * BR_SIZE;
        V3 f0 = ld3(sin.body_f + 6 * gb), t0 = ld3(sin.body_f + 6 * gb + 3);
        for (int k = M.body_joint_start[gb]; k < M.body_joint_start[gb + 1]; ++k) {
            const int e = M.body_joint_entry[k];
            const float* r = drec + (e >> 1) * DR_SIZE;
            if (r[12] != 0.0f) {
                if (e & 1) { f0 += ld3(r + 6); t0 += ld3(r + 9); }
                else { f0 -= ld3(r + 0); t0 -= ld3(r + 3); }
            }
        }
        if ((d.body_flags[gb] & BODY_KINEMATIC) != 0) continue;
        const V3 x0 = ld3(rec + BR_Q);
        const Q4 r0(rec[BR_Q + 3], rec[BR_Q + 4], rec[BR_Q + 5], rec[BR_Q + 6]);
        const V3 v0 = ld3(rec + BR_QD), w0 = ld3(rec + BR_QD + 3);
        const V3 com = ld3(rec + BR_COM);
        const float inv_mass = rec[BR_INVM];
        const M33 inertia = ldm(rec + BR_I);
        const M33 inv_inertia = ldm(rec + BR_INVI);
        int wi = d.body_world[gb];
        if (wi < 0) wi += d.gravity_count;
        const V3 g = ld3(d.gravity + 3 * wi);
        const V3 x_com = x0 + qrot(r0, com);
        const V3 v1 = v0 + (f0 * inv_mass + g * (inv_mass != 0.0f ? 1.0f : 0.0f)) * dt;
        const V3 x1 = x_com + v1 * dt;
        const V3 wb = qrot_inv(r0, w0);
        const V3 tb = qrot_inv(r0, t0) - cross(wb, mv(inertia, wb));
        V3 w1 = qrot(r0, wb + mv(inv_inertia, tb) * dt);
        const Q4 r1 = qunit(qadd(r0, qscale(qscale(qmul(Q4(w1.x, w1.y, w1.z, 0.0f), r0), 0.5f), dt)));
        w1 *= 1.0f - P.angular_damping * dt;
        st3(rec + BR_Q, x1 - qrot(r1, com));
        rec[BR_Q + 3] = r1.x; rec[BR_Q + 4] = r1.y; rec[BR_Q + 5] = r1.z; rec[BR_Q + 6] = r1.w;
        st3(rec + BR_QD, v1);
        st3(rec + BR_QD + 3, w1);
    }
    __syncwarp();
    const size_t T = size_t(M.slot_total);
    const float* cb = M.cb;
    for (int it = 0; it < P.iterations; ++it) {
        const bool sync_it = (flags & XF_PHASE_SYNC) && WARPS > 1, sync_fine = (flags & XF_PHASE_SYNC_FINE) && WARPS > 1;
        if (sync_it) __syncthreads();
        if (use_contacts) {
            for (int c = l; c < nc; c += L) {
                const int s = slot0 + c;
                const int pr = cpair[c];
                const int ba = int(unsigned(pr) & 0x7fffu) - 1, bb = int((unsigned(pr) >> 16) & 0x7fffu) - 1;
                Deltas dl;
                float active = 0.0f;
                if (ba != bb) {
                    const bool need_a = ba >= 0 || want_cimp, need_b = bb >= 0 || want_cimp;
                    BodyView A = ba >= 0 ? load_body(bodies + ba * BR_SIZE) : static_body();
                    BodyView B = bb >= 0 ? load_body(bodies + bb * BR_SIZE) : static_body();
                    const bool cached = c < contact_cache;
                    const float* cc = ccache + c * CC_SIZE;
                    const V3 p0 = cached ? ld3(cc + CC_P0) : V3(cb[CF_P0X * T + s], cb[CF_P0Y * T + s], cb[CF_P0Z * T + s]);
                    const V3 p1 = cached ? ld3(cc + CC_P1) : V3(cb[CF_P1X * T + s], cb[CF_P1Y * T + s], cb[CF_P1Z * T + s]);
                    const V3 n = cached ? ld3(cc + CC_N) : V3(cb[CF_NX * T + s], cb[CF_NY * T + s], cb[CF_NZ * T + s]);
                    V3 bx_a = ba >= 0 ? xpoint(A.X, p0) : V3() + p0, bx_b = bb >= 0 ? xpoint(B.X, p1) : V3() + p1;
                    const float dpen = dot(n, bx_b - bx_a) - (cached ? cc[CC_MSUM] : cb[CF_MARGIN0 * T + s] + cb[CF_MARGIN1 * T + s]);
                    if (dpen < 0.0f) {
                        active = 1.0f;
                        const float mu = cached ? cc[CC_MU] : cb[CF_MU * T + s], mu_t = cached ? cc[CC_MUT] : cb[CF_MU_TORSIONAL * T + s],
                                    mu_r = cached ? cc[CC_MUR] : cb[CF_MU_ROLLING * T + s];
                        const V3 wcom_a = ba >= 0 ? xpoint(A.X, A.com) : V3(), wcom_b = bb >= 0 ? xpoint(B.X, B.com) : V3();
                        V3 r_a = bx_a - wcom_a, r_b = bx_b - wcom_b;
                        V3 ang_a, ang_b;
                        if (need_a) ang_a = -cross(r_a, n);
                        if (need_b) ang_b = cross(r_b, n);
                        const float lambda_n = contact_delta(dpen, A, B, -n, n, ang_a, ang_b, P.rigid_contact_relaxation, dt);
                        V3 lin_da, lin_db, ang_da, ang_db;
                        if (need_a) { lin_da = -n * lambda_n; ang_da = ang_a * lambda_n; }
                        if (need_b) { lin_db = n * lambda_n; ang_db = ang_b * lambda_n; }
                        if (mu > 0.0f) {
                            V3 q0, q1;
                            if (cached) {
                                q0 = ld3(cc + CC_Q0);
                                q1 = ld3(cc + CC_Q1);
                            } else {
                                q0 = p0 + V3(cb[CF_O0X * T + s], cb[CF_O0Y * T + s], cb[CF_O0Z * T + s]);
                                q1 = p1 + V3(cb[CF_O1X * T + s], cb[CF_O1Y * T + s], cb[CF_O1Z * T + s]);
                            }
                            bx_a = ba >= 0 ? xpoint(A.X, q0) : V3() + q0;
                            bx_b = bb >= 0 ? xpoint(B.X, q1) : V3() + q1;
                            V3 delta = bx_b - bx_a;
                            V3 fd = delta - dot(n, delta) * n;
                            r_a = bx_a - wcom_a;
                            r_b = bx_b - wcom_b;
                            V3 rel_v_kin;
                            if (unsigned(pr) & 0x8000u) {
                                V3 v_a = cross(A.w, r_a) + A.v;
                                rel_v_kin = rel_v_kin - (v_a - dot(n, v_a) * n);
                            }
                            if (unsigned(pr) & 0x80000000u) {
                                V3 v_b = cross(B.w, r_b) + B.v;
                                rel_v_kin = rel_v_kin + (v_b - dot(n, v_b) * n);
                            }
                            fd += rel_v_kin * dt;
                            V3 perp = unit(fd);
                            if (need_a) ang_a = -cross(r_a, perp);
                            if (need_b) ang_b = cross(r_b, perp);
                            float err = len(fd);
                            if (err > 0.0f) {
                                float lambda_fr = contact_delta(err, A, B, -perp, perp, ang_a, ang_b, P.rigid_contact_relaxation, dt);
                                lambda_fr = fmax_w(lambda_fr, -lambda_n * mu);
                                if (need_a) { lin_da -= perp * lambda_fr; ang_da += ang_a * lambda_fr; }
                                if (need_b) { lin_db += perp * lambda_fr; ang_db += ang_b * lambda_fr; }
                            }
                        }
                        V3 dom = B.w - A.w;
                        if (mu_t > 0.0f) {
                            float err = dot(dom, n) * dt;
                            if (fabsf(err) > 0.0f) {
                                float lt = contact_delta(err, A, B, V3(), V3(), -n, n, P.rigid_contact_relaxation, dt);
                                lt = clamp_w(lt, -lambda_n * mu_t, lambda_n * mu_t);
                                if (need_a) ang_da -= n * lt;
                                if (need_b) ang_db += n * lt;
                            }
                        }
                        if (mu_r > 0.0f) {
                            dom -= dot(n, dom) * n;
                            float err = len(dom) * dt;
                            if (err > 0.0f) {
                                V3 rn = unit(dom);
                                float lr = contact_delta(err, A, B, V3(), V3(), -rn, rn, P.rigid_contact_relaxation, dt);
                                lr = fmax_w(lr, -lambda_n * mu_r);
                                if (need_a) ang_da -= rn * lr;
                                if (need_b) ang_db += rn * lr;
                            }
                        }
                        dl.lin_p = lin_da;
                        dl.ang_p = ang_da;
                        dl.lin_c = lin_db;
                        dl.ang_c = ang_db;
                    }
                }
                store_deltas(drec + c * DR_SIZE, dl, active);
            }
            __syncwarp();
            if (sync_fine) __syncthreads();
            for (int b = l; b < nb; b += L) {
                V3 dlin, dang;
                float cnt = 0.0f;
                if (use_masks) {
                    unsigned long long m = mask_a | mask_b;
                    while (m) {
                        const int c = __ffsll((long long)m) - 1;
                        m &= m - 1;
                        const float* r = drec + c * DR_SIZE;
                        if (r[12] == 0.0f) continue;
                        if ((mask_a >> c) & 1ull) { dlin += ld3(r + 0); dang += ld3(r + 3); cnt += 1.0f; }
                        if ((mask_b >> c) & 1ull) { dlin += ld3(r + 6); dang += ld3(r + 9); cnt += 1.0f; }
                    }
                } else {
                    for (int c = 0; c < nc; ++c) {
                        const int pr = cpair[c];
                        const int ba = int(unsigned(pr) & 0x7fffu) - 1, bb = int((unsigned(pr) >> 16) & 0x7fffu) - 1;
                        if (ba != b && bb != b) continue;
                        const float* r = drec + c * DR_SIZE;
                        if (r[12] == 0.0f) continue;
                        if (ba == b) { dlin += ld3(r + 0); dang += ld3(r + 3); cnt += 1.0f; }
                        if (bb == b) { dlin += ld3(r + 6); dang += ld3(r + 9); cnt += 1.0f; }
                    }
                }
                apply_delta(bodies + b * BR_SIZE, dlin, dang, cnt, P.rigid_contact_con_weighting != 0, dt);
                if (want_cimp) bcnt[b] = cnt;
            }
            __syncwarp();
            if (want_cimp) {
                for (int c = l; c < nc; c += L) {
                    const float* r = drec + c * DR_SIZE;
                    if (r[12] == 0.0f) continue;
                    const int pr = cpair[c];
                    const int ba = int(unsigned(pr) & 0x7fffu) - 1, bb = int((unsigned(pr) >> 16) & 0x7fffu) - 1;
                    float weight = 1.0f;
                    if (P.rigid_contact_con_weighting) {
                        const float n_a = ba >= 0 ? bcnt[ba] : 0.0f, n_b = bb >= 0 ? bcnt[bb] : 0.0f;
                        const float n_sum = n_a + n_b;
                        if (n_sum > 0.0f) {
                            if (n_a == 0.0f) weight = 1.0f / n_b;
                            else if (n_b == 0.0f) weight = 1.0f / n_a;
                            else weight = 2.0f / n_sum;
                        }
                    }
                    float* ci = M.contact_impulse + slot0 + c;
#pragma unroll
                    for (int k = 0; k < 6; ++k) ci[k * T] = ci[k * T] + r[k] * weight;
                }
                __syncwarp();
            }
        }
        if (d.joint_count > 0) {
            if (sync_fine) __syncthreads();
            for (int j = l; j < nj; j += L) {
                Deltas dl;
                bool act = solve_joint(d, ctl, P, j0 + j, b0, bodies, jcache ? jcache + j * JC_SIZE : nullptr, dt, dl);
                if (!act) dl = Deltas();
                store_deltas(drec + j * DR_SIZE, dl, act ? 1.0f : 0.0f);
                if (want_jimp && act) {
                    float* ji = M.joint_impulse + 6 * size_t(j0 + j);
                    st3(ji, ld3(ji) + dl.lin_c);
                    st3(ji + 3, ld3(ji + 3) + dl.ang_c);
                }
            }
            __syncwarp();
            if (sync_fine) __syncthreads();
            for (int b = l; b < nb; b += L) {
                const int gb = b0 + b;
                V3 dlin, dang;
                for (int k = M.body_joint_start[gb]; k < M.body_joint_start[gb + 1]; ++k) {
                    const int e = M.body_joint_entry[k];
                    const float* r = drec + (e >> 1) * DR_SIZE;
                    if (r[12] == 0.0f) continue;
                    if (e & 1) { dlin += ld3(r + 6); dang += ld3(r + 9); }
                    else { dlin += ld3(r + 0); dang += ld3(r + 3); }
                }
                apply_delta(bodies + b * BR_SIZE, dlin, dang, 0.0f, false, dt);
            }
            __syncwarp();
        }
    }
    if (EX) {
        if (sout.body_parent_f != nullptr) {
            __syncwarp();
            const float inv_dt = 1.0f / dt;
            for (int b = l; b < nb; b += L) {
                const int gb = b0 + b;
                V3 f, t;
                for (int k = M.body_joint_start[gb]; k < M.body_joint_start[gb + 1]; ++k) {
                    const int e = M.body_joint_entry[k];
                    if (!(e & 1)) continue;
                    const int gj = j0 + (e >> 1);
                    if (!d.joint_enabled[gj] || d.joint_type[gj] == JT_FREE) continue;
                    const float* ji = M.joint_impulse + 6 * size_t(gj);
                    f += ld3(ji) * inv_dt;
                    t += ld3(ji + 3) * inv_dt;
                }
                st3(sout.body_parent_f + 6 * gb, f);
                st3(sout.body_parent_f + 6 * gb + 3, t);
            }
        }
        if (P.compute_body_velocity_from_position_delta) {
            for (int b = l; b < nb; b += L) {
                if ((d.body_flags[b0 + b] & BODY_KINEMATIC) != 0) continue;
                float* rec = bodies + b * BR_SIZE;
                const Xf pose = ldx(rec + BR_Q), prev = ldx(init_qd + b * 13);
                const V3 com = ld3(rec + BR_COM);
                const V3 x_com = pose.p + qrot(pose.q, com), x_prev = prev.p + qrot(prev.q, com);
                const V3 v = (x_com - x_prev) / dt;
                const Q4 dq = qmul(pose.q, qconj(prev.q));
                V3 omega = (2.0f / dt) * V3(dq.x, dq.y, dq.z);
                if (dq.w < 0.0f) omega = -omega;
                st3(rec + BR_QD, v);
                st3(rec + BR_QD + 3, omega);
            }
            __syncwarp();
        }
        if (P.enable_restitution && use_contacts) {
            for (int c = l; c < nc; c += L) {
                const int s = slot0 + c;
                const int pr = cpair[c];
                const int ba = int(unsigned(pr) & 0x7fffu) - 1, bb = int((unsigned(pr) >> 16) & 0x7fffu) - 1;
                Deltas dl;
                float active = 0.0f;
                if (ba != bb) {
                    const int sa = __float_as_int(cb[CF_SHAPE0 * T + s]), sb = __float_as_int(cb[CF_SHAPE1 * T + s]);
                    float restitution = 0.0f;
                    restitution += d.shape_material_restitution[sa];
                    restitution += d.shape_material_restitution[sb];
                    restitution /= 2.0f;
                    const float* ra_rec = ba >= 0 ? bodies + ba * BR_SIZE : nullptr;
                    const float* rb_rec = bb >= 0 ? bodies + bb * BR_SIZE : nullptr;
                    const Xf Xa = ba >= 0 ? ldx(init_qd + ba * 13) : Xf(), Xb = bb >= 0 ? ldx(init_qd + bb * 13) : Xf();
                    const V3 com_a = ba >= 0 ? ld3(ra_rec + BR_COM) : V3(), com_b = bb >= 0 ? ld3(rb_rec + BR_COM) : V3();
                    const V3 p0(cb[CF_P0X * T + s], cb[CF_P0Y * T + s], cb[CF_P0Z * T + s]);
                    const V3 p1(cb[CF_P1X * T + s], cb[CF_P1Y * T + s], cb[CF_P1Z * T + s]);
                    const V3 o0(cb[CF_O0X * T + s], cb[CF_O0Y * T + s], cb[CF_O0Z * T + s]);
                    const V3 o1(cb[CF_O1X * T + s], cb[CF_O1Y * T + s], cb[CF_O1Z * T + s]);
                    const V3 n(cb[CF_NX * T + s], cb[CF_NY * T + s], cb[CF_NZ * T + s]);
                    const V3 bx_a = xpoint(Xa, p0 + o0), bx_b = xpoint(Xb, p1 + o1);
                    if (dot(n, bx_b - bx_a) < 0.0f) {
                        const V3 r_a = bx_a - xpoint(Xa, com_a), r_b = bx_b - xpoint(Xb, com_b);
                        V3 v_a, v_b, v_a_new, v_b_new, rxn_a, rxn_b;
                        float inv_mass = 0.0f, m_inv_a = 0.0f, m_inv_b = 0.0f;
                        M33 I_inv_a = m33_zero(), I_inv_b = m33_zero();
                        if (ba >= 0) {
                            int wi = d.body_world[b0 + ba];
                            if (wi < 0) wi += d.gravity_count;
                            m_inv_a = ra_rec[BR_INVM];
                            I_inv_a = ldm(ra_rec + BR_INVI);
                            v_a = (cross(ld3(init_qd + ba * 13 + 10), r_a) + ld3(init_qd + ba * 13 + 7)) + ld3(d.gravity + 3 * wi) * dt;
                            v_a_new = cross(ld3(ra_rec + BR_QD + 3), r_a) + ld3(ra_rec + BR_QD);
                            rxn_a = qrot_inv(Xa.q, cross(r_a, n));
                            inv_mass += m_inv_a + dot(rxn_a, mv(I_inv_a, rxn_a));
                        }
                        if (bb >= 0) {
                            int wi = d.body_world[b0 + bb];
                            if (wi < 0) wi += d.gravity_count;
                            m_inv_b = rb_rec[BR_INVM];
                            I_inv_b = ldm(rb_rec + BR_INVI);
                            v_b = (cross(ld3(init_qd + bb * 13 + 10), r_b) + ld3(init_qd + bb * 13 + 7)) + ld3(d.gravity + 3 * wi) * dt;
                            v_b_new = cross(ld3(rb_rec + BR_QD + 3), r_b) + ld3(rb_rec + BR_QD);
                            rxn_b = qrot_inv(Xb.q, cross(r_b, n));
                            inv_mass += m_inv_b + dot(rxn_b, mv(I_inv_b, rxn_b));
                        }
                        const float rel_old = dot(n, v_b - v_a), rel_new = dot(n, v_b_new - v_a_new);
                        if (inv_mass != 0.0f && rel_old < 0.0f) {
                            const float dv = (-rel_new - restitution * rel_old) / inv_mass;
                            active = 1.0f;
                            if (ba >= 0) {
                                const float dv_a = -dv;
                                dl.lin_p = n * m_inv_a * dv_a;
                                dl.ang_p = qrot(Xa.q, mv(I_inv_a, rxn_a) * dv_a);
                            }
                            if (bb >= 0) {
                                dl.lin_c = n * m_inv_b * dv;
                                dl.ang_c = qrot(Xb.q, mv(I_inv_b, rxn_b) * dv);
                            }
                        }
                    }
                }
                store_deltas(drec + c * DR_SIZE, dl, active);
            }
            __syncwarp();
            for (int b = l; b < nb; b += L) {
                if ((d.body_flags[b0 + b] & BODY_KINEMATIC) != 0) continue;
                V3 dlin, dang;
                for (int c = 0; c < nc; ++c) {
                    const int pr = cpair[c];
                    const int ba = int(unsigned(pr) & 0x7fffu) - 1, bb = int((unsigned(pr) >> 16) & 0x7fffu) - 1;
                    if (ba != b && bb != b) continue;
                    const float* r = drec + c * DR_SIZE;
                    if (r[12] == 0.0f) continue;
                    if (ba == b) { dlin += ld3(r + 0); dang += ld3(r + 3); }
                    if (bb == b) { dlin += ld3(r + 6); dang += ld3(r + 9); }
                }
                float* rec = bodies + b * BR_SIZE;
                st3(rec + BR_QD, ld3(rec + BR_QD) + dlin);
                st3(rec + BR_QD + 3, ld3(rec + BR_QD + 3) + dang);
            }
            __syncwarp();
        }
    }
    if (tma) {
        __syncthreads();
        for (int b = l; b < nb; b += L) {
            const int sb = b0 + b - cb0;
            const float* rec = bodies + b * BR_SIZE;
#pragma unroll
            for (int k = 0; k < 7; ++k) stage[ST_Q * cnb + 7 * sb + k] = rec[BR_Q + k];
#pragma unroll
            for (int k = 0; k < 6; ++k) stage[ST_QD * cnb + 6 * sb + k] = rec[BR_QD + k];
        }
        fence_async_smem();
        __syncthreads();
        if (threadIdx.x == 0) {
            bulk_s2g(sout.body_q + 7 * size_t(cb0), stage + ST_Q * cnb, unsigned(cnb) * 28u);
            bulk_s2g(sout.body_qd + 6 * size_t(cb0), stage + ST_QD * cnb, unsigned(cnb) * 24u);
            bulk_commit_and_drain();
        }
        return;
    }
    for (int b = l; b < nb; b += L) {
        const int gb = b0 + b;
        const float* rec = bodies + b * BR_SIZE;
#pragma unroll
        for (int k = 0; k < 7; ++k) sout.body_q[7 * gb + k] = rec[BR_Q + k];
#pragma unroll
        for (int k = 0; k < 6; ++k) sout.body_qd[6 * gb + k] = rec[BR_QD + k];
    }
}

__global__ void __launch_bounds__(128) xpbd_update_contacts_kernel(DevModel M, nb2_contacts_view out, float inv_dt) {
    const int env = blockIdx.x * (blockDim.x / 32) + (threadIdx.x >> 5);
    if (env >= M.env_count) return;
    const int lane = threadIdx.x & 31;
    const int n = M.env_contact_count[env], base = M.env_contact_offset[env], slot0 = M.env_slot_start[env];
    const size_t T = size_t(M.slot_total);
    for (int c = lane; c < n; c += 32) {
        int o = base + c;
        if (o >= out.rigid_contact_max) break;
        if (M.export_rank) o = M.export_rank[o];
#pragma unroll
        for (int k = 0; k < 6; ++k) out.force[6 * size_t(o) + k] = M.contact_impulse[k * T + slot0 + c] * inv_dt;
    }
}

__global__ void __launch_bounds__(256) integrate_bodies_kernel(nb2_model_desc d, nb2_state_view sin, nb2_state_view sout,
                                                                float angular_damping, float dt) {
    const int b = blockIdx.x * blockDim.x + threadIdx.x;
    if (b >= d.body_count) return;
    Xf X = ldx(sin.body_q + 7 * b);
    V3 v0 = ld3(sin.body_qd + 6 * b), w0 = ld3(sin.body_qd + 6 * b + 3);
    if ((d.body_flags[b] & BODY_KINEMATIC) != 0) {
        stx(sout.body_q + 7 * b, X);
        st3(sout.body_qd + 6 * b, v0);
        st3(sout.body_qd + 6 * b + 3, w0);
        return;
    }
    V3 f0 = ld3(sin.body_f + 6 * b), t0 = ld3(sin.body_f + 6 * b + 3);
    const V3 com = ld3(d.body_com + 3 * b);
    const float inv_mass = d.body_inv_mass[b];
    const M33 inertia = ldm(d.body_inertia + 9 * b), inv_inertia = ldm(d.body_inv_inertia + 9 * b);
    int wi = d.body_world[b];
    if (wi < 0) wi += d.gravity_count;
    const V3 g = ld3(d.gravity + 3 * wi);
    const V3 x_com = X.p + qrot(X.q, com);
    const V3 v1 = v0 + (f0 * inv_mass + g * (inv_mass != 0.0f ? 1.0f : 0.0f)) * dt;
    const V3 x1 = x_com + v1 * dt;
    const V3 wb = qrot_inv(X.q, w0);
    const V3 tb = qrot_inv(X.q, t0) - cross(wb, mv(inertia, wb));
    V3 w1 = qrot(X.q, wb + mv(inv_inertia, tb) * dt);
    const Q4 r1 = qunit(qadd(X.q, qscale(qscale(qmul(Q4(w1.x, w1.y, w1.z, 0.0f), X.q), 0.5f), dt)));
    w1 *= 1.0f - angular_damping * dt;
    stx(sout.body_q + 7 * b, Xf(x1 - qrot(r1, com), r1));
    st3(sout.body_qd + 6 * b, v1);
    st3(sout.body_qd + 6 * b + 3, w1);
}

static int env_int(const char* name, int fallback) {
    const char* v = std::getenv(name);
    return v ? std::atoi(v) : fallback;
}

template <int L, bool EX, int WARPS>
static nb2_status launch_xpbd_W(nb2_model* m, const nb2_xpbd_params& p, const nb2_state_view& in, const nb2_state_view& out,
                                const nb2_control_view& ctl, int use_contacts, float dt, cudaStream_t s) {
    const DevModel& M = m->dev;
    constexpr int NE = (32 / L) * WARPS;
    const int blocks = (M.env_count + NE - 1) / NE;
    const int contact_cap = m->contacts_imported ? M.max_env_contact_slots : std::min(M.max_env_contact_slots, m->max_env_contacts);
    if (M.max_env_bodies > 32000) {
        set_error("xpbd_step: environment too large for the fused shared-memory kernel (bodies per env)");
        return NB2_ERR_CAPACITY;
    }
    static const bool cache_enabled = std::getenv("NB2_XPBD_NO_JOINT_CACHE") == nullptr;
    static const int tma_enabled = env_int("NB2_XPBD_TMA", 1), phase_sync = env_int("NB2_XPBD_PHASE_SYNC", 1);
    int flags = (tma_enabled ? XF_TMA : 0) | (phase_sync >= 1 ? XF_PHASE_SYNC : 0) | (phase_sync >= 2 ? XF_PHASE_SYNC_FINE : 0);
    XpbdPlan plan = xpbd_plan(NE, M.max_env_bodies, M.max_env_joints, contact_cap, EX, false);
    if (cache_enabled && M.d.joint_count > 0) {
        const XpbdPlan with_cache = xpbd_plan(NE, M.max_env_bodies, M.max_env_joints, contact_cap, EX, true);
        const int want_ctas = (16 + WARPS - 1) / WARPS;
        if ((size_t(with_cache.total) * sizeof(float) + 1024) * want_ctas <= 227 * 1024 || size_t(plan.total) * sizeof(float) * want_ctas > 227 * 1024) {
            if (size_t(with_cache.total) * sizeof(float) <= 220 * 1024) {
                plan = with_cache;
                flags |= XF_JOINT_CACHE;
            }
        }
    }
    int contact_cache = 0;
    {
        static const int cc_enabled = env_int("NB2_XPBD_CONTACT_CACHE", 1);
        const int want_ctas = (16 + WARPS - 1) / WARPS;
        const size_t budget = (size_t(227) * 1024) / want_ctas - 1024 - 64;
        const size_t base = size_t(plan.total) * sizeof(float);
        if (cc_enabled && use_contacts && base < budget) {
            contact_cache = int(std::min<size_t>((budget - base) / (size_t(NE) * CC_SIZE * sizeof(float)), size_t(contact_cap)));
            if (contact_cache > 0)
                plan = xpbd_plan(NE, M.max_env_bodies, M.max_env_joints, contact_cap, EX, (flags & XF_JOINT_CACHE) != 0, contact_cache);
        }
    }
    const size_t smem = size_t(plan.total) * sizeof(float);
    if (smem > 220 * 1024 + 6 * 1024) {
        set_error("xpbd_step: environment too large for the fused shared-memory kernel (bodies/contacts per env)");
        return NB2_ERR_CAPACITY;
    }
    if (smem > 48 * 1024)
        NB2_CUDA_CHECK(cudaFuncSetAttribute(xpbd_step_kernel<L, EX, WARPS>, cudaFuncAttributeMaxDynamicSharedMemorySize, int(smem)));
    static const int carveout = std::getenv("NB2_XPBD_CARVEOUT") ? std::atoi(std::getenv("NB2_XPBD_CARVEOUT")) : int(cudaSharedmemCarveoutMaxShared);
    NB2_CUDA_CHECK(cudaFuncSetAttribute(xpbd_step_kernel<L, EX, WARPS>, cudaFuncAttributePreferredSharedMemoryCarveout, carveout));
    static const int min_grid = env_int("NB2_XPBD_MIN_GRID", 0);
    const int grid = blocks < min_grid ? min_grid : blocks;
    xpbd_step_kernel<L, EX, WARPS><<<grid, 32 * WARPS, smem, s>>>(M, p, in, out, ctl, use_contacts, dt, flags, contact_cap, contact_cache);
    count_launch();
    NB2_CUDA_CHECK(cudaGetLastError());
    return NB2_OK;
}

template <int L, bool EX>
static nb2_status launch_xpbd_L(nb2_model* m, const nb2_xpbd_params& p, const nb2_state_view& in, const nb2_state_view& out,
                                const nb2_control_view& ctl, int use_contacts, float dt, cudaStream_t s) {
    static const int forced = env_int("NB2_XPBD_WARPS", 0);
    int warps = forced;
    if (warps <= 0) {
        int sms = 132;
        cudaDeviceGetAttribute(&sms, cudaDevAttrMultiProcessorCount, m->device);
        const long long total_warps = (m->dev.env_count + (32 / L) - 1) / (32 / L);
        const long long per_sm = (total_warps + sms - 1) / sms;
        warps = per_sm <= 1 ? 1 : (per_sm <= 4 ? 4 : 16);
    }
    auto fits = [&](int w) {
        const int ne = (32 / L) * w;
        const int cap = m->contacts_imported ? m->dev.max_env_contact_slots : std::min(m->dev.max_env_contact_slots, m->max_env_contacts);
        return size_t(xpbd_plan(ne, m->dev.max_env_bodies, m->dev.max_env_joints, cap, EX, false).total) * sizeof(float) <= 200 * 1024;
    };
    if (warps >= 16 && !fits(16)) warps = 4;
    if (warps >= 4 && warps < 16 && !fits(4)) warps = 1;
#ifdef NB2_XPBD_AB_VARIANTS
    if constexpr (L == 16 && !EX) {
        if (warps == 2) return launch_xpbd_W<L, EX, 2>(m, p, in, out, ctl, use_contacts, dt, s);
        if (warps == 7) return launch_xpbd_W<L, EX, 7>(m, p, in, out, ctl, use_contacts, dt, s);
    }
#endif
    if (warps >= 16) return launch_xpbd_W<L, EX, 16>(m, p, in, out, ctl, use_contacts, dt, s);
    if (warps >= 4) return launch_xpbd_W<L, EX, 4>(m, p, in, out, ctl, use_contacts, dt, s);
    return launch_xpbd_W<L, EX, 1>(m, p, in, out, ctl, use_contacts, dt, s);
}

nb2_status launch_xpbd_step(nb2_model* m, const nb2_xpbd_params& p, const nb2_state_view& in, const nb2_state_view& out,
                            const nb2_control_view& ctl, int use_contacts, float dt, cudaStream_t s) {
    const DevModel& M = m->dev;
    if (M.d.body_count == 0) return NB2_OK;
    if (!in.body_q || !in.body_qd || !in.body_f || !out.body_q || !out.body_qd) {
        set_error("nb2_xpbd_step: state arrays are NULL");
        return NB2_ERR_INVALID_ARGUMENT;
    }
    if (M.d.joint_count > 0 && (!ctl.joint_f || !ctl.joint_target_q || !ctl.joint_target_qd)) {
        set_error("nb2_xpbd_step: control arrays are NULL");
        return NB2_ERR_INVALID_ARGUMENT;
    }
    if (p.enable_restitution && !M.d.shape_material_restitution) {
        set_error("nb2_xpbd_step: enable_restitution needs model.shape_material_restitution");
        return NB2_ERR_INVALID_ARGUMENT;
    }
    const bool ex = p.enable_restitution || p.compute_body_velocity_from_position_delta || out.body_parent_f != nullptr ||
                    ((use_contacts & NB2_XPBD_CONTACT_IMPULSE) && (use_contacts & NB2_XPBD_USE_CONTACTS));
#define NB2_XPBD_DISPATCH(LANES)                                                                        \
    return ex ? launch_xpbd_L<LANES, true>(m, p, in, out, ctl, use_contacts, dt, s)                     \
              : launch_xpbd_L<LANES, false>(m, p, in, out, ctl, use_contacts, dt, s)
    switch (m->lanes_per_env) {
        case 8: NB2_XPBD_DISPATCH(8);
        case 16: NB2_XPBD_DISPATCH(16);
        default: NB2_XPBD_DISPATCH(32);
    }
#undef NB2_XPBD_DISPATCH
}

nb2_status launch_xpbd_update_contacts(nb2_model* m, const nb2_contacts_view& contacts, cudaStream_t s) {
    const DevModel& M = m->dev;
    NB2_CUDA_CHECK(cudaMemsetAsync(contacts.force, 0, size_t(contacts.rigid_contact_max) * 6 * sizeof(float), s));
    if (M.env_count == 0) return NB2_OK;
    xpbd_update_contacts_kernel<<<(M.env_count + 3) / 4, 128, 0, s>>>(M, contacts, 1.0f / m->xpbd_impulse_dt);
    count_launch();
    NB2_CUDA_CHECK(cudaGetLastError());
    return NB2_OK;
}

nb2_status launch_integrate_bodies(nb2_model* m, const nb2_state_view& in, const nb2_state_view& out, float angular_damping, float dt,
                                   cudaStream_t s) {
    const nb2_model_desc& d = m->dev.d;
    if (d.body_count == 0) return NB2_OK;
    integrate_bodies_kernel<<<(d.body_count + 255) / 256, 256, 0, s>>>(d, in, out, angular_damping, dt);
    count_launch();
    NB2_CUDA_CHECK(cudaGetLastError());
    return NB2_OK;
}

}
```

Before: 19.51 million.

## Spill excess XPBD contacts to global overflow buffer and use joint bitmasks

Shared memory for contacts is now sized to a fitted count K. Contacts beyond K keep their pair and delta records in a new global overflow buffer instead of shared memory. The contact cache fill moves after body staging, and warp-count selection no longer counts contacts, so larger warp configurations become eligible. Per-body joint accumulation now uses per-lane bitmasks instead of CSR lookups when joints per env are at most 64. The trade-off is global-memory traffic and extra branching for overflow contacts in exchange for higher occupancy.

```diff
diff --git a/newton_b200/build.py b/newton_b200/build.py
--- a/newton_b200/build.py
+++ b/newton_b200/build.py
@@ -57,12 +57,12 @@
     return LIB
 
 
-def build_variant(tag: str, defines: list[str], strict: bool = True, sources=None) -> str:
-    lib_path = os.path.join(HERE, f"libnewton_b200_{tag}.so")
+def build_variant(tag: str, defines: list[str], strict: bool = True, sources=None, out_dir: str | None = None) -> str:
+    lib_path = os.path.join(out_dir or HERE, f"libnewton_b200_{tag}.so")
     flags = NVCC_FLAGS + (STRICT_FLAGS if strict else []) + list(defines)
     procs, objs = [], []
     for src in SOURCES:
-        obj = os.path.join(CSRC, src.replace(".cu", f".{tag}.o"))
+        obj = os.path.join(out_dir or CSRC, src.replace(".cu", f".{tag}.o"))
         objs.append(obj)
         procs.append((src, subprocess.Popen([_nvcc(), *flags, "-c", os.path.join(CSRC, src), "-o", obj], stdout=subprocess.PIPE,
                                             stderr=subprocess.STDOUT, text=True)))
diff --git a/newton_b200/csrc/nb2_api.cu b/newton_b200/csrc/nb2_api.cu
--- a/newton_b200/csrc/nb2_api.cu
+++ b/newton_b200/csrc/nb2_api.cu
@@ -446,6 +446,9 @@
     NB2_CUDA_CHECK(cudaMemset(p, 0, cb_bytes));
     m->allocations.push_back(p);
     dv.cb = static_cast<float*>(p);
+    NB2_CUDA_CHECK(cudaMalloc(&p, std::max<size_t>(size_t(dv.slot_total) * 14, 1) * sizeof(float)));
+    m->allocations.push_back(p);
+    dv.xpbd_overflow = static_cast<float*>(p);
     NB2_CUDA_CHECK(cudaMalloc(&p, (size_t(dv.env_count) + 1) * sizeof(int)));
     NB2_CUDA_CHECK(cudaMemset(p, 0, (size_t(dv.env_count) + 1) * sizeof(int)));
     m->allocations.push_back(p);
@@ -484,6 +487,7 @@
     release(m, dv.env_slot_start);
     release(m, dv.cb);
     release(m, dv.contact_impulse);
+    release(m, dv.xpbd_overflow);
     dv.max_env_contact_slots = 0;
     for (int e = 0; e < E; ++e) dv.max_env_contact_slots = std::max(dv.max_env_contact_slots, h.env_slot_start[e + 1] - h.env_slot_start[e]);
     dv.slot_total = h.env_slot_start[E];
@@ -500,6 +504,9 @@
     NB2_CUDA_CHECK(cudaMemset(p, 0, n));
     m->allocations.push_back(p);
     dv.cb = static_cast<float*>(p);
+    NB2_CUDA_CHECK(cudaMalloc(&p, std::max<size_t>(size_t(dv.slot_total) * 14, 1) * sizeof(float)));
+    m->allocations.push_back(p);
+    dv.xpbd_overflow = static_cast<float*>(p);
     NB2_CUDA_CHECK(cudaMemset(dv.env_contact_count, 0, (size_t(E) + 1) * sizeof(int)));
     return NB2_OK;
 }
diff --git a/newton_b200/csrc/nb2_internal.cuh b/newton_b200/csrc/nb2_internal.cuh
--- a/newton_b200/csrc/nb2_internal.cuh
+++ b/newton_b200/csrc/nb2_internal.cuh
@@ -40,6 +40,7 @@
     const int* body_joint_start;
     const int* body_joint_entry;
     float* cb;
+    float* xpbd_overflow;
     int slot_total;
     int* env_contact_count;
     int* env_contact_offset;
diff --git a/newton_b200/csrc/nb2_xpbd.cu b/newton_b200/csrc/nb2_xpbd.cu
--- a/newton_b200/csrc/nb2_xpbd.cu
+++ b/newton_b200/csrc/nb2_xpbd.cu
@@ -445,19 +445,19 @@
 NB2_GPU void fence_async_smem() { asm volatile("fence.proxy.async.shared::cta;" ::: "memory"); }
 
 struct XpbdPlan {
-    int bodies, jcache, cpair, ccache, extra, drec, mbar, total;
+    int bodies, jcache, cpair, extra, ccache, drec, mbar, total;
     int rec_cap;
 };
-__host__ __device__ inline XpbdPlan xpbd_plan(int NE, int MB, int MJ, int CC, bool ex, bool joint_cache, int contact_cache = 0) {
+__host__ __device__ inline XpbdPlan xpbd_plan(int NE, int MB, int MJ, int K, bool ex, bool joint_cache) {
     XpbdPlan o;
     auto up4 = [](int x) { return (x + 3) & ~3; };
-    o.rec_cap = MB > MJ ? (MB > CC ? MB : CC) : (MJ > CC ? MJ : CC);
+    o.rec_cap = MB > MJ ? (MB > K ? MB : K) : (MJ > K ? MJ : K);
     o.bodies = 0;
     o.jcache = up4(o.bodies + NE * MB * BR_SIZE);
     o.cpair = up4(o.jcache + (joint_cache ? NE * MJ * JC_SIZE : 0));
-    o.ccache = up4(o.cpair + NE * CC);
-    o.extra = up4(o.ccache + NE * contact_cache * CC_SIZE);
-    o.drec = up4(o.extra + (ex ? NE * MB * 14 : 0));
+    o.extra = up4(o.cpair + NE * K);
+    o.ccache = up4(o.extra + (ex ? NE * MB * 14 : 0));
+    o.drec = up4(o.ccache + NE * K * CC_SIZE);
     o.mbar = up4(o.drec + NE * o.rec_cap * DR_SIZE);
     o.total = o.mbar + 4;
     return o;
@@ -470,7 +470,7 @@
 template <int L, bool EX, int WARPS>
 __global__ void __launch_bounds__(32 * WARPS, (WARPS >= NB2_XPBD_MIN_WARPS ? 1 : NB2_XPBD_MIN_WARPS / WARPS))
 xpbd_step_kernel(DevModel M, nb2_xpbd_params P, nb2_state_view sin, nb2_state_view sout, nb2_control_view ctl, int use_contacts_flags,
-                 float dt, int flags, int contact_cap, int contact_cache) {
+                 float dt, int flags, int contact_cap, int K) {
     const int use_contacts = use_contacts_flags & NB2_XPBD_USE_CONTACTS;
     const bool want_cimp = EX && use_contacts && (use_contacts_flags & NB2_XPBD_CONTACT_IMPULSE);
     const bool want_jimp = EX && sout.body_parent_f != nullptr;
@@ -487,15 +487,15 @@
     const int env = env0 + slot;
     const bool live = env < M.env_count;
     const nb2_model_desc& d = M.d;
-    const XpbdPlan plan = xpbd_plan(NE, M.max_env_bodies, M.max_env_joints, contact_cap, EX, joint_cache, contact_cache);
-    float* ccache = smem + plan.ccache + slot * contact_cache * CC_SIZE;
+    const XpbdPlan plan = xpbd_plan(NE, M.max_env_bodies, M.max_env_joints, K, EX, joint_cache);
+    float* ccache = smem + plan.ccache + slot * K * CC_SIZE;
     float* bodies = smem + plan.bodies + slot * M.max_env_bodies * BR_SIZE;
     float* drec = smem + plan.drec + slot * plan.rec_cap * DR_SIZE;
-    int* cpair = reinterpret_cast<int*>(smem + plan.cpair) + slot * contact_cap;
+    int* cpair = reinterpret_cast<int*>(smem + plan.cpair) + slot * K;
     float* init_qd = smem + plan.extra + slot * M.max_env_bodies * 14;
     float* bcnt = init_qd + M.max_env_bodies * 13;
     float* jcache = joint_cache ? smem + plan.jcache + slot * M.max_env_joints * JC_SIZE : nullptr;
-    float* stage = smem + plan.drec;
+    float* stage = smem + plan.ccache;
     unsigned long long* mbar = reinterpret_cast<unsigned long long*>(smem + plan.mbar);
 
     int b0 = 0, nb = 0, j0 = 0, nj = 0, slot0 = 0, nc = 0;
@@ -507,9 +507,12 @@
         slot0 = M.env_slot_start[env];
         nc = use_contacts ? min(M.env_contact_count[env], contact_cap) : 0;
     }
+    float* ovf = M.xpbd_overflow + 14 * size_t(slot0);
+    auto contact_pair = [&](int c) { return c < K ? cpair[c] : __float_as_int(ovf[14 * c + 13]); };
+    auto contact_rec = [&](int c) -> float* { return c < K ? drec + c * DR_SIZE : ovf + 14 * c; };
     const int env_last = min(env0 + NE, M.env_count);
     const int cb0 = M.env_body_start[env0], cnb = M.env_body_start[env_last] - cb0;
-    bool tma = (flags & XF_TMA) != 0 && cnb > 0 && (cb0 & 3) == 0 && (cnb & 3) == 0 && cnb * ST_PER_BODY <= NE * plan.rec_cap * DR_SIZE;
+    bool tma = (flags & XF_TMA) != 0 && cnb > 0 && (cb0 & 3) == 0 && (cnb & 3) == 0 && cnb * ST_PER_BODY <= plan.mbar - plan.ccache;
     if (tma) {
         const uintptr_t a = reinterpret_cast<uintptr_t>(sin.body_q) | reinterpret_cast<uintptr_t>(sin.body_qd) |
                             reinterpret_cast<uintptr_t>(sout.body_q) | reinterpret_cast<uintptr_t>(sout.body_qd) |
@@ -534,24 +537,9 @@
         const size_t T = size_t(M.slot_total);
         int ba = __float_as_int(M.cb[CF_BODY_A * T + slot0 + c]), bb = __float_as_int(M.cb[CF_BODY_B * T + slot0 + c]);
         const unsigned ka = ba >= 0 && (d.body_flags[b0 + ba] & BODY_KINEMATIC) != 0, kb = bb >= 0 && (d.body_flags[b0 + bb] & BODY_KINEMATIC) != 0;
-        cpair[c] = int(unsigned(ba + 1) | (ka << 15) | (unsigned(bb + 1) << 16) | (kb << 31));
-        if (c < contact_cache) {
-            const int s = slot0 + c;
-            float* cc = ccache + c * CC_SIZE;
-            const V3 p0(M.cb[CF_P0X * T + s], M.cb[CF_P0Y * T + s], M.cb[CF_P0Z * T + s]);
-            const V3 p1(M.cb[CF_P1X * T + s], M.cb[CF_P1Y * T + s], M.cb[CF_P1Z * T + s]);
-            const V3 o0(M.cb[CF_O0X * T + s], M.cb[CF_O0Y * T + s], M.cb[CF_O0Z * T + s]);
-            const V3 o1(M.cb[CF_O1X * T + s], M.cb[CF_O1Y * T + s], M.cb[CF_O1Z * T + s]);
-            st3(cc + CC_P0, p0);
-            st3(cc + CC_P1, p1);
-            st3(cc + CC_N, V3(M.cb[CF_NX * T + s], M.cb[CF_NY * T + s], M.cb[CF_NZ * T + s]));
-            cc[CC_MSUM] = M.cb[CF_MARGIN0 * T + s] + M.cb[CF_MARGIN1 * T + s];
-            cc[CC_MU] = M.cb[CF_MU * T + s];
-            cc[CC_MUT] = M.cb[CF_MU_TORSIONAL * T + s];
-            cc[CC_MUR] = M.cb[CF_MU_ROLLING * T + s];
-            st3(cc + CC_Q0, p0 + o0);
-            st3(cc + CC_Q1, p1 + o1);
-        }
+        const int pr = int(unsigned(ba + 1) | (ka << 15) | (unsigned(bb + 1) << 16) | (kb << 31));
+        if (c < K) cpair[c] = pr;
+        else ovf[14 * c + 13] = __int_as_float(pr);
         if (want_cimp)
 #pragma unroll
             for (int k = 0; k < 6; ++k) M.contact_impulse[k * T + slot0 + c] = 0.0f;
@@ -610,16 +598,43 @@
 #pragma unroll
             for (int k = 0; k < 13; ++k) init_qd[b * 13 + k] = bodies[b * BR_SIZE + BR_Q + k];
     if (tma) __syncthreads();
-    else __syncwarp();
+    for (int c = l; c < min(nc, K); c += L) {
+        const size_t T = size_t(M.slot_total);
+        const int s = slot0 + c;
+        float* cc = ccache + c * CC_SIZE;
+        const V3 p0(M.cb[CF_P0X * T + s], M.cb[CF_P0Y * T + s], M.cb[CF_P0Z * T + s]);
+        const V3 p1(M.cb[CF_P1X * T + s], M.cb[CF_P1Y * T + s], M.cb[CF_P1Z * T + s]);
+        const V3 o0(M.cb[CF_O0X * T + s], M.cb[CF_O0Y * T + s], M.cb[CF_O0Z * T + s]);
+        const V3 o1(M.cb[CF_O1X * T + s], M.cb[CF_O1Y * T + s], M.cb[CF_O1Z * T + s]);
+        st3(cc + CC_P0, p0);
+        st3(cc + CC_P1, p1);
+        st3(cc + CC_N, V3(M.cb[CF_NX * T + s], M.cb[CF_NY * T + s], M.cb[CF_NZ * T + s]));
+        cc[CC_MSUM] = M.cb[CF_MARGIN0 * T + s] + M.cb[CF_MARGIN1 * T + s];
+        cc[CC_MU] = M.cb[CF_MU * T + s];
+        cc[CC_MUT] = M.cb[CF_MU_TORSIONAL * T + s];
+        cc[CC_MUR] = M.cb[CF_MU_ROLLING * T + s];
+        st3(cc + CC_Q0, p0 + o0);
+        st3(cc + CC_Q1, p1 + o1);
+    }
+    __syncwarp();
     const bool use_masks = nb <= L && nc <= 64;
     unsigned long long mask_a = 0ull, mask_b = 0ull;
     if (use_masks && l < nb)
         for (int c = 0; c < nc; ++c) {
-            const int pr = cpair[c];
+            const int pr = contact_pair(c);
             const int ba = int(unsigned(pr) & 0x7fffu) - 1, bb = int((unsigned(pr) >> 16) & 0x7fffu) - 1;
             if (ba == bb) continue;
             if (ba == l) mask_a |= 1ull << c;
             if (bb == l) mask_b |= 1ull << c;
+        }
+    const bool use_jmasks = nb <= L && nj <= 64;
+    unsigned long long jmask_p = 0ull, jmask_c = 0ull;
+    if (use_jmasks && l < nb)
+        for (int j = 0; j < nj; ++j) {
+            const int p = jcache ? jc_int(jcache + j * JC_SIZE, JC_PARENT) : d.joint_parent[j0 + j];
+            const int ch = jcache ? jc_int(jcache + j * JC_SIZE, JC_CHILD) : d.joint_child[j0 + j];
+            if (p >= 0 && p - b0 == l) jmask_p |= 1ull << j;
+            if (ch - b0 == l) jmask_c |= 1ull << j;
         }
     for (int j = l; j < nj; j += L) {
         Deltas w;
@@ -638,12 +653,24 @@
         const int gb = b0 + b;
         float* rec = bodies + b * BR_SIZE;
         V3 f0 = ld3(sin.body_f + 6 * gb), t0 = ld3(sin.body_f + 6 * gb + 3);
-        for (int k = M.body_joint_start[gb]; k < M.body_joint_start[gb + 1]; ++k) {
-            const int e = M.body_joint_entry[k];
-            const float* r = drec + (e >> 1) * DR_SIZE;
-            if (r[12] != 0.0f) {
-                if (e & 1) { f0 += ld3(r + 6); t0 += ld3(r + 9); }
-                else { f0 -= ld3(r + 0); t0 -= ld3(r + 3); }
+        if (use_jmasks) {
+            unsigned long long m = jmask_p | jmask_c;
+            while (m) {
+                const int j = __ffsll((long long)m) - 1;
+                m &= m - 1;
+                const float* r = drec + j * DR_SIZE;
+                if (r[12] == 0.0f) continue;
+                if ((jmask_p >> j) & 1ull) { f0 -= ld3(r + 0); t0 -= ld3(r + 3); }
+                if ((jmask_c >> j) & 1ull) { f0 += ld3(r + 6); t0 += ld3(r + 9); }
+            }
+        } else {
+            for (int k = M.body_joint_start[gb]; k < M.body_joint_start[gb + 1]; ++k) {
+                const int e = M.body_joint_entry[k];
+                const float* r = drec + (e >> 1) * DR_SIZE;
+                if (r[12] != 0.0f) {
+                    if (e & 1) { f0 += ld3(r + 6); t0 += ld3(r + 9); }
+                    else { f0 -= ld3(r + 0); t0 -= ld3(r + 3); }
+                }
             }
         }
         if ((d.body_flags[gb] & BODY_KINEMATIC) != 0) continue;
@@ -679,7 +706,8 @@
         if (use_contacts) {
             for (int c = l; c < nc; c += L) {
                 const int s = slot0 + c;
-                const int pr = cpair[c];
+                const bool cached = c < K;
+                const int pr = contact_pair(c);
                 const int ba = int(unsigned(pr) & 0x7fffu) - 1, bb = int((unsigned(pr) >> 16) & 0x7fffu) - 1;
                 Deltas dl;
                 float active = 0.0f;
@@ -687,7 +715,6 @@
                     const bool need_a = ba >= 0 || want_cimp, need_b = bb >= 0 || want_cimp;
                     BodyView A = ba >= 0 ? load_body(bodies + ba * BR_SIZE) : static_body();
                     BodyView B = bb >= 0 ? load_body(bodies + bb * BR_SIZE) : static_body();
-                    const bool cached = c < contact_cache;
                     const float* cc = ccache + c * CC_SIZE;
                     const V3 p0 = cached ? ld3(cc + CC_P0) : V3(cb[CF_P0X * T + s], cb[CF_P0Y * T + s], cb[CF_P0Z * T + s]);
                     const V3 p1 = cached ? ld3(cc + CC_P1) : V3(cb[CF_P1X * T + s], cb[CF_P1Y * T + s], cb[CF_P1Z * T + s]);
@@ -770,32 +797,36 @@
                         dl.ang_c = ang_db;
                     }
                 }
-                store_deltas(drec + c * DR_SIZE, dl, active);
+                if (cached) store_deltas(drec + c * DR_SIZE, dl, active);
+                else store_deltas(ovf + 14 * c, dl, active);
             }
             __syncwarp();
             if (sync_fine) __syncthreads();
             for (int b = l; b < nb; b += L) {
                 V3 dlin, dang;
                 float cnt = 0.0f;
+                auto add = [&](const float* r, bool side_a, bool side_b) {
+                    if (r[12] == 0.0f) return;
+                    if (side_a) { dlin += ld3(r + 0); dang += ld3(r + 3); cnt += 1.0f; }
+                    if (side_b) { dlin += ld3(r + 6); dang += ld3(r + 9); cnt += 1.0f; }
+                };
                 if (use_masks) {
-                    unsigned long long m = mask_a | mask_b;
-                    while (m) {
+                    const unsigned long long all = mask_a | mask_b, shared = K >= 64 ? all : all & ((1ull << K) - 1ull);
+                    for (unsigned long long m = shared; m; m &= m - 1) {
                         const int c = __ffsll((long long)m) - 1;
-                        m &= m - 1;
-                        const float* r = drec + c * DR_SIZE;
-                        if (r[12] == 0.0f) continue;
-                        if ((mask_a >> c) & 1ull) { dlin += ld3(r + 0); dang += ld3(r + 3); cnt += 1.0f; }
-                        if ((mask_b >> c) & 1ull) { dlin += ld3(r + 6); dang += ld3(r + 9); cnt += 1.0f; }
+                        add(drec + c * DR_SIZE, (mask_a >> c) & 1ull, (mask_b >> c) & 1ull);
+                    }
+                    for (unsigned long long m = all & ~shared; m; m &= m - 1) {
+                        const int c = __ffsll((long long)m) - 1;
+                        add(ovf + 14 * c, (mask_a >> c) & 1ull, (mask_b >> c) & 1ull);
                     }
                 } else {
                     for (int c = 0; c < nc; ++c) {
-                        const int pr = cpair[c];
+                        const int pr = contact_pair(c);
                         const int ba = int(unsigned(pr) & 0x7fffu) - 1, bb = int((unsigned(pr) >> 16) & 0x7fffu) - 1;
                         if (ba != b && bb != b) continue;
-                        const float* r = drec + c * DR_SIZE;
-                        if (r[12] == 0.0f) continue;
-                        if (ba == b) { dlin += ld3(r + 0); dang += ld3(r + 3); cnt += 1.0f; }
-                        if (bb == b) { dlin += ld3(r + 6); dang += ld3(r + 9); cnt += 1.0f; }
+                        if (c < K) add(drec + c * DR_SIZE, ba == b, bb == b);
+                        else add(ovf + 14 * c, ba == b, bb == b);
                     }
                 }
                 apply_delta(bodies + b * BR_SIZE, dlin, dang, cnt, P.rigid_contact_con_weighting != 0, dt);
@@ -804,9 +835,9 @@
             __syncwarp();
             if (want_cimp) {
                 for (int c = l; c < nc; c += L) {
-                    const float* r = drec + c * DR_SIZE;
+                    const float* r = contact_rec(c);
                     if (r[12] == 0.0f) continue;
-                    const int pr = cpair[c];
+                    const int pr = contact_pair(c);
                     const int ba = int(unsigned(pr) & 0x7fffu) - 1, bb = int((unsigned(pr) >> 16) & 0x7fffu) - 1;
                     float weight = 1.0f;
                     if (P.rigid_contact_con_weighting) {
@@ -843,12 +874,24 @@
             for (int b = l; b < nb; b += L) {
                 const int gb = b0 + b;
                 V3 dlin, dang;
-                for (int k = M.body_joint_start[gb]; k < M.body_joint_start[gb + 1]; ++k) {
-                    const int e = M.body_joint_entry[k];
-                    const float* r = drec + (e >> 1) * DR_SIZE;
-                    if (r[12] == 0.0f) continue;
-                    if (e & 1) { dlin += ld3(r + 6); dang += ld3(r + 9); }
-                    else { dlin += ld3(r + 0); dang += ld3(r + 3); }
+                if (use_jmasks) {
+                    unsigned long long m = jmask_p | jmask_c;
+                    while (m) {
+                        const int j = __ffsll((long long)m) - 1;
+                        m &= m - 1;
+                        const float* r = drec + j * DR_SIZE;
+                        if (r[12] == 0.0f) continue;
+                        if ((jmask_p >> j) & 1ull) { dlin += ld3(r + 0); dang += ld3(r + 3); }
+                        if ((jmask_c >> j) & 1ull) { dlin += ld3(r + 6); dang += ld3(r + 9); }
+                    }
+                } else {
+                    for (int k = M.body_joint_start[gb]; k < M.body_joint_start[gb + 1]; ++k) {
+                        const int e = M.body_joint_entry[k];
+                        const float* r = drec + (e >> 1) * DR_SIZE;
+                        if (r[12] == 0.0f) continue;
+                        if (e & 1) { dlin += ld3(r + 6); dang += ld3(r + 9); }
+                        else { dlin += ld3(r + 0); dang += ld3(r + 3); }
+                    }
                 }
                 apply_delta(bodies + b * BR_SIZE, dlin, dang, 0.0f, false, dt);
             }
@@ -894,12 +937,12 @@
         if (P.enable_restitution && use_contacts) {
             for (int c = l; c < nc; c += L) {
                 const int s = slot0 + c;
-                const int pr = cpair[c];
+                const int pr = contact_pair(c);
                 const int ba = int(unsigned(pr) & 0x7fffu) - 1, bb = int((unsigned(pr) >> 16) & 0x7fffu) - 1;
                 Deltas dl;
                 float active = 0.0f;
                 if (ba != bb) {
-                    const int sa = __float_as_int(cb[CF_SHAPE0 * T + s]), sb = __float_as_int(cb[CF_SHAPE1 * T + s]);
+                    const int sa =__float_as_int(cb[CF_SHAPE0 * T + s]), sb = __float_as_int(cb[CF_SHAPE1 * T + s]);
                     float restitution = 0.0f;
                     restitution += d.shape_material_restitution[sa];
                     restitution += d.shape_material_restitution[sb];
@@ -955,17 +998,17 @@
                         }
                     }
                 }
-                store_deltas(drec + c * DR_SIZE, dl, active);
+                store_deltas(contact_rec(c), dl, active);
             }
             __syncwarp();
             for (int b = l; b < nb; b += L) {
                 if ((d.body_flags[b0 + b] & BODY_KINEMATIC) != 0) continue;
                 V3 dlin, dang;
                 for (int c = 0; c < nc; ++c) {
-                    const int pr = cpair[c];
+                    const int pr = contact_pair(c);
                     const int ba = int(unsigned(pr) & 0x7fffu) - 1, bb = int((unsigned(pr) >> 16) & 0x7fffu) - 1;
                     if (ba != b && bb != b) continue;
-                    const float* r = drec + c * DR_SIZE;
+                    const float* r = contact_rec(c);
                     if (r[12] == 0.0f) continue;
                     if (ba == b) { dlin += ld3(r + 0); dang += ld3(r + 3); }
                     if (bb == b) { dlin += ld3(r + 6); dang += ld3(r + 9); }
@@ -1058,6 +1101,13 @@
     return v ? std::atoi(v) : fallback;
 }
 
+#ifdef NB2_XPBD_TEST_CONTACT_K
+static int g_test_last_contact_k = -1;
+}
+extern "C" int nb2_xpbd_test_last_contact_k(void) { return nb2::g_test_last_contact_k; }
+namespace nb2 {
+#endif
+
 template <int L, bool EX, int WARPS>
 static nb2_status launch_xpbd_W(nb2_model* m, const nb2_xpbd_params& p, const nb2_state_view& in, const nb2_state_view& out,
                                 const nb2_control_view& ctl, int use_contacts, float dt, cudaStream_t s) {
@@ -1072,41 +1122,35 @@
     static const bool cache_enabled = std::getenv("NB2_XPBD_NO_JOINT_CACHE") == nullptr;
     static const int tma_enabled = env_int("NB2_XPBD_TMA", 1), phase_sync = env_int("NB2_XPBD_PHASE_SYNC", 1);
     int flags = (tma_enabled ? XF_TMA : 0) | (phase_sync >= 1 ? XF_PHASE_SYNC : 0) | (phase_sync >= 2 ? XF_PHASE_SYNC_FINE : 0);
-    XpbdPlan plan = xpbd_plan(NE, M.max_env_bodies, M.max_env_joints, contact_cap, EX, false);
-    if (cache_enabled && M.d.joint_count > 0) {
-        const XpbdPlan with_cache = xpbd_plan(NE, M.max_env_bodies, M.max_env_joints, contact_cap, EX, true);
-        const int want_ctas = (16 + WARPS - 1) / WARPS;
-        if ((size_t(with_cache.total) * sizeof(float) + 1024) * want_ctas <= 227 * 1024 || size_t(plan.total) * sizeof(float) * want_ctas > 227 * 1024) {
-            if (size_t(with_cache.total) * sizeof(float) <= 220 * 1024) {
-                plan = with_cache;
-                flags |= XF_JOINT_CACHE;
-            }
-        }
-    }
-    int contact_cache = 0;
-    {
-        static const int cc_enabled = env_int("NB2_XPBD_CONTACT_CACHE", 1);
-        const int want_ctas = (16 + WARPS - 1) / WARPS;
-        const size_t budget = (size_t(227) * 1024) / want_ctas - 1024 - 64;
-        const size_t base = size_t(plan.total) * sizeof(float);
-        if (cc_enabled && use_contacts && base < budget) {
-            contact_cache = int(std::min<size_t>((budget - base) / (size_t(NE) * CC_SIZE * sizeof(float)), size_t(contact_cap)));
-            if (contact_cache > 0)
-                plan = xpbd_plan(NE, M.max_env_bodies, M.max_env_joints, contact_cap, EX, (flags & XF_JOINT_CACHE) != 0, contact_cache);
-        }
-    }
-    const size_t smem = size_t(plan.total) * sizeof(float);
-    if (smem > 220 * 1024 + 6 * 1024) {
-        set_error("xpbd_step: environment too large for the fused shared-memory kernel (bodies/contacts per env)");
+    auto plan_bytes = [&](int k, bool jcache) { return size_t(xpbd_plan(NE, M.max_env_bodies, M.max_env_joints, k, EX, jcache).total) * sizeof(float); };
+    const int want_ctas = (16 + WARPS - 1) / WARPS;
+    const size_t resident = (size_t(227) * 1024) / want_ctas - 1024 - 64;
+    const size_t budget = plan_bytes(0, false) <= resident ? resident : size_t(220 + 6) * 1024;
+    auto fit_k = [&](bool jcache) {
+        int k = contact_cap;
+        while (k >= 0 && plan_bytes(k, jcache) > budget) --k;
+        return k;
+    };
+    const int k_floor = std::min(contact_cap, std::max(M.max_env_bodies, M.max_env_joints));
+    const bool jcache = cache_enabled && M.d.joint_count > 0 && fit_k(true) >= k_floor;
+    if (jcache) flags |= XF_JOINT_CACHE;
+    int K = fit_k(jcache);
+#ifdef NB2_XPBD_TEST_CONTACT_K
+    K = std::min(K, NB2_XPBD_TEST_CONTACT_K);
+    g_test_last_contact_k = K;
+#endif
+    if (K < 0) {
+        set_error("xpbd_step: environment too large for the fused shared-memory kernel (bodies/joints per env)");
         return NB2_ERR_CAPACITY;
     }
+    const size_t smem = plan_bytes(K, jcache);
     if (smem > 48 * 1024)
         NB2_CUDA_CHECK(cudaFuncSetAttribute(xpbd_step_kernel<L, EX, WARPS>, cudaFuncAttributeMaxDynamicSharedMemorySize, int(smem)));
     static const int carveout = std::getenv("NB2_XPBD_CARVEOUT") ? std::atoi(std::getenv("NB2_XPBD_CARVEOUT")) : int(cudaSharedmemCarveoutMaxShared);
     NB2_CUDA_CHECK(cudaFuncSetAttribute(xpbd_step_kernel<L, EX, WARPS>, cudaFuncAttributePreferredSharedMemoryCarveout, carveout));
     static const int min_grid = env_int("NB2_XPBD_MIN_GRID", 0);
     const int grid = blocks < min_grid ? min_grid : blocks;
-    xpbd_step_kernel<L, EX, WARPS><<<grid, 32 * WARPS, smem, s>>>(M, p, in, out, ctl, use_contacts, dt, flags, contact_cap, contact_cache);
+    xpbd_step_kernel<L, EX, WARPS><<<grid, 32 * WARPS, smem, s>>>(M, p, in, out, ctl, use_contacts, dt, flags, contact_cap, K);
     count_launch();
     NB2_CUDA_CHECK(cudaGetLastError());
     return NB2_OK;
@@ -1126,8 +1170,7 @@
     }
     auto fits = [&](int w) {
         const int ne = (32 / L) * w;
-        const int cap = m->contacts_imported ? m->dev.max_env_contact_slots : std::min(m->dev.max_env_contact_slots, m->max_env_contacts);
-        return size_t(xpbd_plan(ne, m->dev.max_env_bodies, m->dev.max_env_joints, cap, EX, false).total) * sizeof(float) <= 200 * 1024;
+        return size_t(xpbd_plan(ne, m->dev.max_env_bodies, m->dev.max_env_joints, 0, EX, false).total) * sizeof(float) <= 200 * 1024;
     };
     if (warps >= 16 && !fits(16)) warps = 4;
     if (warps >= 4 && warps < 16 && !fits(4)) warps = 1;
```

Result: no change. 19.58 million, median of 6 (+0.4%).
